# dfdazac/grapes

Measured on AMD Instinct MI355X. Metric: sampled edges aggregated/sec, ogbn-products 3-layer GFlowNet, higher is better.
Workload: dtype f32

## Files before the change

### grapes_amd/_lib.py

```python
from __future__ import annotations

import ctypes as C
import os

_HERE = os.path.dirname(os.path.abspath(__file__))
DIAG_LIB_PATH = os.path.join(_HERE, "libgrapes_hip_diag.so")
DIAG = os.environ.get("GRAPES_DIAG", "0") == "1"
LIB_PATH = os.environ.get("GRAPES_LIB_PATH") or (DIAG_LIB_PATH if DIAG else os.path.join(_HERE, "libgrapes_hip.so"))
ABI_MAJOR, ABI_MINOR = 3, 4


def diag_switch(name: str, default: str) -> str:
    if os.environ.get("GRAPES_DIAG", "0") == "1":
        return os.environ.get(name, default)
    return default


P = C.c_void_p
I32 = C.c_int32
I64 = C.c_int64
U32 = C.c_uint32
U64 = C.c_uint64
F32 = C.c_float
SZ = C.c_size_t
# ... 117 lines not shown
    "grapes_gcn2_mix_fwd": (I32, [P, P, P, F32, F32, F32, I32, P, I32, P, I32, P]),
    "grapes_gcn2_mix_bwd": (I32, [P, P, I32, F32, F32, F32, P, P, P, I32, P, I32, P]),
    "grapes_wgcn_structure_workspace_bytes": (SZ, [I32]),
    "grapes_wgcn_structure": (I32, [P, P, I32, P, I32, P] + [P] * 12),
    "grapes_wgcn_weights": (I32, [P, I32] + [P] * 7 + [I32, P, I32, F32] + [P] * 5),
    "grapes_wgcn_aggregate_workspace_bytes": (SZ, [I32, I32]),
    "grapes_wgcn_aggregate_fwd": (I32, [P] * 8 + [I32, P, I32, I32, I32, P, P, I32, P, P, P]),
    "grapes_wgcn_aggregate_bwd_workspace_bytes": (SZ, [I32, I32, I32, I32]),
    "grapes_wgcn_aggregate_bwd": (I32, [P] * 5 + [I32] + [P] * 14 + [I32, P, I32, I32, P, P, P, P, I32, P, P, P]),
    "grapes_wgcn_loops_workspace_bytes": (SZ, [I32, I32]),
    "grapes_wgcn_loops": (I32, [P, P, I32, P, I32, P, P, P, P, P]),
    "grapes_pna_aggregate_fwd_workspace_bytes": (SZ, [I32, I32]),
    "grapes_pna_aggregate_fwd": (I32, [P, P, P, I32, P, P, P, I32, I32, I32, I32, F32, F32, P, P, I32, P, I32, P, P, I32, P, P, P]),
    "grapes_pna_aggregate_bwd_workspace_bytes": (SZ, [I32, I32, I32]),
    "grapes_pna_aggregate_bwd": (I32, [P, P, I32, P, P, P, P, P, I32, I32, I32, I32, F32, F32, P, P, I32, I32, P, I32, P, P, I32, P, P, P]),
    "grapes_pna_add_input_grad": (I32, [P, P, I32, I32, P, I32, P]),
    "grapes_kernel_clock_enable": (I32, [P, I64]),
    "grapes_kernel_clock_launches": (I32, []),
    "grapes_kernel_clock_entry": (I32, [I32, P, P, P]),
    "grapes_kernel_clock_rate_khz": (I32, []),
    "grapes_gcn_aggregate_fwd_rec": (I32, [P, P, P, P, P, P, P, I32, P, I32, I32, P, P, P, P]),
    "grapes_scatter_rows": (I32, [P, I64, P, P, I64, I32, I32, P, I32, I32, P]),
    "grapes_rider_record_begin": (I32, []),
    "grapes_rider_record_end": (I32, []),
    "grapes_rider_count": (I32, [I32]),
    "grapes_rider_attach": (I32, [I32, I32, P]),
    "grapes_rider_release": (I32, [P]),
    "grapes_rider_detach": (I32, [P, P]),
    "grapes_rider_launch": (I32, [I32, P]),
    "grapes_rider_free": (I32, [I32]),
    "grapes_graph_chain_create": (I32, [P, I32, I32, P, P]),
    "grapes_graph_chain_launch": (I32, [P, P]),
    "grapes_graph_chain_destroy": (I32, [P]),
    "grapes_tensormap_update": (I32, [P, P, I32, P, P]),
    "grapes_tensormap_map": (I32, [P, P, P, I64, P, P]),
    "grapes_frontier_offsets": (I32, [P, P, I32, P, P, P, P]),
    "grapes_frontier_expand": (I32, [P, P, P, I32, P, P, I32, P, P, P, P, P]),
    "grapes_frontier_expand_fused": (I32, [P, P, P, I32, P, I32, P, P, P, P, P, P, P, I32, P, P, P, P, P]),
    "grapes_frontier_expand_fused_ext": (I32, [P, P, P, I32, P, I32, P, P, P, P, P, P, P, I32, P, P, P, P, P, P, P, P, P]),
    "grapes_slice_stage_words": (SZ, [I32]),
    "grapes_bitmap_mark": (I32, [P, P, P, I64, P, I32, P, P]),
    "grapes_bitmap_mark_rows": (I32, [P, P, P, I32, P, P, I32, P, P]),
    "grapes_bitmap_clear": (I32, [P, P, I64, P, P]),
    "grapes_frontier_compact_workspace_bytes": (SZ, [I32, I32]),
    "grapes_frontier_compact": (I32, [P, P, P, I32, I32, P, P, P, P, P, P, U32, P, I32, P, P, SZ, P, SZ, P, SZ, P, P, P, P, P]),
    "grapes_frontier_compact_counted": (I32, [P, P, P, I32, I32, P, P, P, P, P, P, U32, P, I32, P, P, SZ, P, SZ, P, SZ, P, P, P, P, P, P]),
    "grapes_gcn_prepare_counted": (I32, [P, P, P, I32, P, P, I32, P, P, P, P, P, P, P, P, P, P, P, P, P, I64, I32, P, P]),
    "grapes_bitmap_mark_hop": (I32, [P, P, P, P, I32, P, P, P, I32, P, I32, P, P]),
    "grapes_bitmap_mark_lists": (I32, [P, P, P, I32, P, P, I32, P, P, I32, P, P, I32, P, I32, P, P, P]),
    "grapes_union_sorted": (I32, [P, I32, P, P, I32, P, P, I32, P, P, I32, P, I32, I32, P, P, P, P, P, P]),
    "grapes_slice_mark": (I32, [P, P, I32, P, I32, P, P]),
    "grapes_slice_remark": (I32, [P, P, I32, P, P, I32, P, P, P, I32, P, P]),
    "grapes_slice_filter_workspace_bytes": (SZ, [I32]),
    "grapes_slice_filter": (I32, [P, P, P, I32, P, I32, P, P, P, P, P, I32, P, P]),
    "grapes_indicator_mark": (I32, [P, P, I32, P, U32, P, I32, I32, P]),
    "grapes_step_begin": (I32, [P, P, I32, P, I32, P, I32, I32, I32, P, P, I32, I32, P, P]),
    "grapes_gather_rows": (I32, [P, I32, P, I32, P, P, U32, P, I32, P, P]),
    "grapes_gcn_prepare_workspace_bytes": (SZ, [I32, I32]),
    "grapes_gcn_prepare_zero_words": (SZ, [I32]),
    "grapes_gcn_long_items_capacity": (I32, [I32]),
    "grapes_gcn_prepare": (I32, [P, P, I32, P, P, I32, P, I32, P, P, P, P, P, P, P, P, P, P, P, P, P]),
    "grapes_gcn_prepare_prefetching": (I32, [P, P, I32, P, P, I32, P, I32, P, P, P, P, P, P, P, P, P, P, P, P, P, I64, I32, P]),
    "grapes_gcn_prepare_small_batch": (I32, [I32, P, P, P, P, P, I32, P, P, P, P, P, P, P, P, P, P, P, P, P, P, P, P]),
    "grapes_gcn_prepare_from_csr": (I32, [P, I32, P, P, P, I32, P]),
    "grapes_linear_fwd": (I32, [P, P, P, I32, P, I32, I32, P]),
    "grapes_linear_fwd_row_scaled": (I32, [P, P, P, P, I32, P, I32, I32, P]),
    "grapes_eval_predict": (I32, [P, I32, I32, P, P, I32, P, P, P, P]),
    "grapes_linear_bwd_weight_workspace_bytes": (SZ, [I32, I32, I32]),
    "grapes_linear_bwd_weight": (I32, [P, P, P, I32, P, I32, I32, I32, P, P]),
    "grapes_linear_bwd_input": (I32, [P, P, P, I32, P, I32, I32, P]),
    "grapes_linear_bias_act_fwd": (I32, [P, P, P, I32, P, I32, P, I32, I32, P]),
    "grapes_linear_bias_act_head_fwd": (I32, [P, P, P, I32, P, P, P, I32, P, I32, I32, P]),
    "grapes_split_gemm_available": (I32, [I32, I32, I32]),
    "grapes_sampler_head_bwd_multi_workspace_bytes": (SZ, []),
    "grapes_sampler_head_bwd_multi_phase": (I32, [I32, P, P, P, P, P, P, P, P, P, P, P, P, I32, P, P, P, I32, P]),
    "grapes_linear_bias_act_head_fwd_strided": (I32, [P, I32, P, P, I32, P, P, P, I32, P, I32, I32, P]),
    "grapes_linear_bwd_weight_gated_strided": (I32, [P, P, I32, P, I32, P, P, P, P, P, I32, I32, I32, P, P]),
    "grapes_linear_bwd_weight_gated_workspace_bytes": (SZ, [I32, I32, I32]),
    "grapes_linear_bwd_weight_gated": (I32, [P, P, P, P, P, I32, P, I32, I32, I32, P, P, P, P, P]),
    "grapes_linear_bwd_weight_gated_multi": (I32, [I32, P, P, P, P, P, P, P, P, P, I32, I32, I32, P, P]),
    "grapes_linear_bwd_weight_slabs_bytes": (SZ, [I32, I32, I32]),
    "grapes_linear_bwd_weight_slabs": (I32, [P, P, P, I32, P, I32, I32, I32, P, P]),
    "grapes_linear_bwd_weight_slabs_and_input": (I32, [P, P, P, P, P, I32, P, I32, I32, I32, P, P]),
    "grapes_slab_reduce_sets": (I32, [I32, P, P, P, I32, P, I32, P]),
    "grapes_gcn_aggregate_narrow_pair": (I32, [P, P, P, P, P, P, P, P, P, I32, P, P]),
    "grapes_linear_relu_head_fwd_bits": (I32, [P, I32, P, P, P, P, P, I32, P, I32, I32, P]),
    "grapes_linear_relu_head_fwd_bits_pair": (I32, [P, I32, P, P, P, P, P, P, I32, P, P, P, P, P, I32, I32, P, I32, I32, P]),
    "grapes_linear_bwd_weight_bits_multi_cols": (I32, [I32, P, P, P, P, P, P, P, P, P, P, I32, P, P, I32, I32, I32, P, P]),
    "grapes_linear_bwd_weight_bits_pair_cols": (I32, [I32, P, P, P, P, P, P, P, P, P, P, I32, P, P, I32, P, P, P, P, P, P, I32, I32, I32, P, P]),
    "grapes_gcn_aggregate_gather_fwd": (I32, [P, I32, I32, P, P, U32, P, I32, P, P, P, P, P, I32, P, P]),
    "grapes_gcn_aggregate_gather_fwd_peers": (I32, [P, P, I32, I32, I32, P, P, U32, P, I32, P, P, P, P, P, I32, P, P]),
    "grapes_peer_export": (I32, [P, P, P]),
    "grapes_peer_open": (I32, [P, U64, P]),
    "grapes_peer_close": (I32, [P, U64]),
    "grapes_peer_copy": (I32, [P, P, SZ, P]),
    "grapes_gcn_aggregate_workspace_bytes": (SZ, [I32, I32]),
    "grapes_gcn_aggregate_fwd": (I32, [P, P, P, P, P, P, I32, P, I32, I32, P, P, I32, P, P]),
    "grapes_gcn_aggregate_fwd_head": (I32, [P, P, P, P, P, P, I32, P, I32, I32, P, P, P, P]),
    "grapes_gcn_aggregate_fwd_prescaled": (I32, [P, P, P, P, P, P, I32, P, I32, I32, P, P, I32, P, P]),
    "grapes_scale_rows": (I32, [P, P, P, I64, I32, P]),
    "grapes_gcn_aggregate_bwd_rank1_workspace_bytes": (SZ, [I32, I32]),
    "grapes_gcn_aggregate_bwd_rank1": (I32, [P, P, P, P, P, P, P, P, P, I32, I32, P, I32, P, P, I32, P, P]),
    "grapes_gcn_aggregate_bwd_rank1_bits": (I32, [P, P, P, P, P, P, P, P, P, P, I32, I32, P, I32, P, P, I32, P, P]),
    "grapes_gcn_aggregate_bwd_rank1_bits_multi": (I32, [I32, P, P, P, P, P, P, P, P, P, P, P, P, P, I32, P, P, P, P, P]),
    "grapes_gcn_aggregate_bwd_workspace_bytes": (SZ, [I32, I32]),
    "grapes_gcn_aggregate_bwd": (I32, [P, P, P, P, P, P, P, P, I32, I32, P, I32, P, P, I32, P, P, P]),
    "grapes_sampler_workspace_bytes": (SZ, [I32]),
    "grapes_gumbel_topk": (I32, [P, P, P, U64, U64, P, I32, P, I32, I32, P, P, P, P, P, P, P, P, P, I32, P, P, P, P]),
    "grapes_gumbel_topk_hist": (I32, [P, P, P, U64, U64, P, I32, P, I32, I32, P, P, P, P, P, P, P, P, P, I32, P, P, P, P, P]),
    "grapes_gumbel_topk_deferred_ext": (I32, [P, P, P, U64, U64, P, I32, P, I32, I32, P, P, P, P, P, P, P, P, P, I32, P, P, P, P, P, P, P, P, P]),
    "grapes_sampler_hist_words": (I32, []),
    "grapes_gumbel_topk_from_aggregate": (I32, [P, P, P, P, P, P, I32, P, P, P, P, U64, U64, P, I32, P, I32, I32, P, P, P, P, P, P, P, P, P, I32, P, P, P, P]),
    "grapes_bernoulli_logprob_bwd": (I32, [P, P, P, P, P, P, I32, P, P, I32, P, P, P]),
    "grapes_philox_uniform": (I32, [P, I64, U64, U64, P]),
    "grapes_reduce_sum": (I32, [P, I32, P, I32, P, P]),
    "grapes_fill": (I32, [P, I32, P, F32, P, F32, P, I32, P]),
    "grapes_classifier_loss": (I32, [P, I32, I32, P, P, P, P, I32, P, P, P]),
    "grapes_gflownet_loss": (I32, [P, F32, P, I32, I32, P, F32, I32, P, P]),
    "grapes_step_losses_workspace_bytes": (SZ, [I32]),
    "grapes_step_losses": (I32, [P, I32, I32, P, P, P, P, I32, P, P, P, I32, P, F32, P, I32, I32, F32, I32, P, P, P, P, P]),
    "grapes_gcn_aggregate_fwd_losses_available": (I32, [P, P, P, I32, I32]),
    "grapes_gcn_aggregate_fwd_losses": (I32, [P, P, P, P, P, P, I32, P, I32, P, P, P, P, I32, P, P, P, I32, P, F32, P, I32, I32, F32,
                                              I32, P, P, P, P]),
    "grapes_logit_var_reg": (I32, [P, I32, P, I32, F32, P, P, P]),
    "grapes_dropout_fwd": (I32, [P, P, P, I32, P, I32, F32, U64, U64, P, P]),
    "grapes_dropout_bwd": (I32, [P, P, P, I32, P, I32, F32, P]),
    "grapes_adam_desc_bytes": (I32, []),
    "grapes_adam_step": (I32, [P, I32, I64, P, P]),
    "grapes_adam_step_slabs": (I32, [P, I32, I64, P, I32, P, P, I32, P, I32, P]),
    "grapes_exchange_pack_query": (I32, [P, I32, P, I32, P, P]),
    "grapes_exchange_serve_rows": (I32, [P, P, P, I32, I32, I32, I32, P, I64, I32, P, P, P]),
    "grapes_exchange_recv_rows": (I32, [P, I64, P, I32, P, P, I32, I32, P, P, P, P, P, P, P]),
    "grapes_exchange_serve_features": (I32, [P, I32, P, I32, I32, I32, I32, P, I32, P, P]),
    "grapes_exchange_assemble_features": (I32, [P, I32, I32, P, I32, P, P, I32, P, U32, P, I32, P, P]),
    "grapes_exchange_halo_positions": (I32, [P, I32, P, P, I32, I32, P, P, P, P]),
    "grapes_exchange_note_rows": (I32, [P, P, I32, P, P, P, I32, P, P, P, P, I32, P]),
}

_lib = None


DIAG_SIGNATURES = {
    "grapes_debug_gemm_fwd": (I32, [P, P, P, I32, I32, I32, I32, P]),
    "grapes_debug_gather_probe": (I32, [P, I32, P, P, I32, I32, I32, I32, P]),
    "grapes_debug_tsplit_fwd": (I32, [P, I32, I32, P, P, P, I32, I32, I32, P]),
    "grapes_debug_tsplit_dw": (I32, [P, P, I32, I32, P, I32, I32, P, I32, P]),
    "grapes_feature_planes_bytes": (C.c_size_t, [I64, I32]),
    "grapes_feature_split_planes": (I32, [P, I64, I32, P, P]),
    "grapes_feature_planes_register": (I32, [P, I32, P]),
}


class GrapesHipError(RuntimeError):
    pass


_diag_lib = None


def _bind(lib, table, what):
    for name, (res, args) in table.items():
        try:
            fn = getattr(lib, name)
        except AttributeError as e:
            raise GrapesHipError(f"{what} does not export {name}") from e
        fn.restype = res
        fn.argtypes = args


def load_diag():
    global _diag_lib
    if _diag_lib is not None:
        return _diag_lib
    if _lib is not None and LIB_PATH == DIAG_LIB_PATH:
        _diag_lib = _lib
        return _diag_lib
    if not os.path.exists(DIAG_LIB_PATH):
        raise GrapesHipError(f"{DIAG_LIB_PATH} is missing: build it with `make -C grapes_amd/csrc diag`")
    lib = C.CDLL(DIAG_LIB_PATH)
    _bind(lib, SIGNATURES, "libgrapes_hip_diag.so")
    _bind(lib, DIAG_SIGNATURES, "libgrapes_hip_diag.so")
    if lib.grapes_build_flavor() != b"diag":
        raise GrapesHipError("libgrapes_hip_diag.so was not built with -DGRAPES_DIAG")
    _diag_lib = lib
    return lib


def load():
    global _lib
# ... 22 lines not shown
```

### grapes_amd/csrc/common.h

```cpp
#pragma once
#include <hip/hip_runtime.h>
#include <stdint.h>

#include "../../include/grapes_hip.h"

#define GRAPES_WAVE 64
#define DWS_ROWS 128

#define GRAPES_LAUNCH_CHECK()                      \
    do {                                           \
        hipError_t _e = hipGetLastError();         \
        if (_e != hipSuccess) return (int)_e;      \
    } while (0)

static inline int grapes_div_up(int64_t a, int64_t b) { return (int)((a + b - 1) / b); }
static inline bool grapes_aligned16(const void* p) { return (((uintptr_t)p) & 15) == 0; }
static inline size_t grapes_round16(size_t b) { return (b + 15) & ~(size_t)15; }

#include <stdlib.h>
static inline const char* grapes_tune_env(const char* name) {
#ifdef GRAPES_DIAG
    return getenv(name);
#else
    (void)name;
// ... 257 lines not shown
#define GRAPES_STAMP_NW(slot)                                                                                \
    do {                                                                                                     \
        if (grapes_stamp_ptr && threadIdx.x == 0 && blockIdx.x < 64)                                         \
            grapes_stamp_ptr[blockIdx.x * 16 + (slot)] = wall_clock64();                                      \
    } while (0)
#define GRAPES_STAMP_SETTER(name)                                                                            \
    extern "C" int name(unsigned long long* p) {                                                             \
        return (int)hipMemcpyToSymbol(HIP_SYMBOL(grapes_stamp_ptr), &p, sizeof(p));                          \
    }
#else
#define GRAPES_STAMP(slot) do { } while (0)
#define GRAPES_STAMP_NW(slot) do { } while (0)
#define GRAPES_STAMP_SETTER(name)
#endif

#define GRAPES_TS_IMG_ROWS 256

#ifdef __HIPCC__
template <int NT>
__device__ __forceinline__ void draw_stats_final(const double* __restrict__ parts, int blocks, int n, float* __restrict__ stats) {
    __shared__ double ds_red[4][16];
    const int tid = threadIdx.x, lane = tid & 63, wid = tid >> 6;
#pragma unroll
    for (int q = 0; q < 1024 / NT; ++q) {
        double mn = (double)INFINITY, mx = -(double)INFINITY, s1 = 0.0, s2 = 0.0;
        for (int b = tid + NT * q; b < blocks; b += 1024) {
            const long long* p = reinterpret_cast<const long long*>(parts + 5 * (size_t)b);
            mn = fmin(mn, __longlong_as_double(__hip_atomic_load(p + 0, __ATOMIC_RELAXED, __HIP_MEMORY_SCOPE_AGENT)));
            mx = fmax(mx, __longlong_as_double(__hip_atomic_load(p + 1, __ATOMIC_RELAXED, __HIP_MEMORY_SCOPE_AGENT)));
            s1 += __longlong_as_double(__hip_atomic_load(p + 2, __ATOMIC_RELAXED, __HIP_MEMORY_SCOPE_AGENT));
            s2 += __longlong_as_double(__hip_atomic_load(p + 3, __ATOMIC_RELAXED, __HIP_MEMORY_SCOPE_AGENT));
        }
#pragma unroll
        for (int d = 32; d > 0; d >>= 1) {
            mn = fmin(mn, __shfl_xor(mn, d, 64)); mx = fmax(mx, __shfl_xor(mx, d, 64));
            s1 += __shfl_xor(s1, d, 64); s2 += __shfl_xor(s2, d, 64);
        }
        if (lane == 0) { const int vw = wid + (NT / 64) * q; ds_red[0][vw] = mn; ds_red[1][vw] = mx; ds_red[2][vw] = s1; ds_red[3][vw] = s2; }
    }
    __syncthreads();
    if (tid == 0) {
        double mn = (double)INFINITY, mx = -(double)INFINITY, s1 = 0.0, s2 = 0.0;
        for (int w = 0; w < 16; ++w) { mn = fmin(mn, ds_red[0][w]); mx = fmax(mx, ds_red[1][w]); s1 += ds_red[2][w]; s2 += ds_red[3][w]; }
        const double mean = s1 / (double)n;
        double var = n > 1 ? (s2 - s1 * s1 / (double)n) / (double)(n - 1) : 0.0;
        if (var < 0.0) var = 0.0;
        stats[0] = (float)mn; stats[1] = (float)mx; stats[2] = (float)mean; stats[3] = (float)sqrt(var);
    }
}
__device__ __forceinline__ void draw_finish_body(const grapes_draw_finish_args& f) {
    __shared__ double df_red[16];
    const int tid = threadIdx.x, lane = tid & 63, wid = tid >> 6;
    const int n = eff_count(f.d_n, f.n_host);
    const bool keep_all = f.sel[2] != 0u;
    const int nb = keep_all ? f.keys_blocks : (n + f.emit_block - 1) / f.emit_block;
    const double* parts = keep_all ? f.parts_keys : f.parts_emit;
    const int pstride = keep_all ? 5 : 1;
    double v[4];
#pragma unroll
    for (int q = 0; q < 4; ++q) {
        double acc = 0.0;
        for (int bb = tid + 256 * q; bb < nb; bb += 1024) acc += parts[(size_t)bb * pstride];
        v[q] = acc;
    }
#pragma unroll
    for (int q = 0; q < 4; ++q) { const double w = wave_sum_d(v[q]); if (lane == 0) df_red[wid + 4 * q] = w; }
    __syncthreads();
    if (tid == 0 && f.stats) {
        double t = 0.0;
        for (int w = 0; w < 16; ++w) t += df_red[w];
        f.stats[4] = (float)t;
    }
    if (f.hist)
        for (int b = tid; b < f.hist_words; b += 256) f.hist[b] = 0u;
    if (f.stats_blocks > 0 && !keep_all && f.stats) draw_stats_final<256>(f.parts_keys - 4, nb, n, f.stats);
}
#endif

#include <functional>
#include <type_traits>
#include <string.h>
enum GrapesRiderKind { GRAPES_RK_OTHER = 0, GRAPES_RK_EXPAND, GRAPES_RK_COMPACT, GRAPES_RK_FILL, GRAPES_RK_SORT, GRAPES_RK_GATHER,
                       GRAPES_RK_BEGIN ,
                       GRAPES_RK_AGGBWD  };
struct GrapesRiderRecord {
    int kind = GRAPES_RK_OTHER, variant = 0, grid = 0, block = 0;
    size_t arg_bytes = 0;
    alignas(16) unsigned char args[768];
    std::function<void(hipStream_t)> single;
};
bool grapes_rider_recording();
int grapes_rider_grid(int grid);
void grapes_rider_record(GrapesRiderRecord&& r);
#define GRAPES_RIDER_ANY_VARIANT (-0x7fffffff)
const GrapesRiderRecord* grapes_rider_match(int kind, int variant, int block, hipStream_t s);
template <class Args>
static inline GrapesRiderRecord grapes_rider_make(int kind, int variant, int grid, int block, const Args& a,
                                                  std::function<void(hipStream_t)> single) {
    static_assert(sizeof(Args) <= sizeof(GrapesRiderRecord::args), "rider argument block too small");
    static_assert(std::is_trivially_copyable<Args>::value, "rider arguments must be trivially copyable");
    GrapesRiderRecord r;
    r.kind = kind; r.variant = variant; r.grid = grid; r.block = block; r.arg_bytes = sizeof(Args);
    memcpy(r.args, &a, sizeof(Args));
    r.single = std::move(single);
    return r;
}
#define GRAPES_RIDER_OTHER(stream_, launch_expr_)                                                                         \
    do {                                                                                                                  \
        if (grapes_rider_recording()) {                                                                                   \
            GrapesRiderRecord r_;                                                                                         \
            r_.single = [=](hipStream_t s_) { hipStream_t stream_ = s_; (void)stream_; launch_expr_; };                   \
            grapes_rider_record(std::move(r_));                                                                           \
        } else {                                                                                                          \
            launch_expr_;                                                                                                 \
        }                                                                                                                 \
    } while (0)
```

### grapes_amd/csrc/gemm_kernels.hip

```cpp
#include <type_traits>
#include "common.h"
#include <cstdlib>

typedef float f32x16 __attribute__((ext_vector_type(16)));

#define GB_M 128
#define GB_N 128
#define GB_K 16
#define GB_LD 132

struct GatherOp { const int32_t* ids; const uint32_t* code; const uint32_t* d_epoch; uint32_t epoch; int F; uint32_t mask; };

template <bool KMAJOR, bool VEC>
__device__ __forceinline__ void gemm_load_tile(const float* __restrict__ P, long long ld, int r0, int R, int k0,
                                               int kend, int tid, float4 (&v)[2], const float* __restrict__ G = nullptr,
                                               int ones_at = -1, const float* __restrict__ row_scale = nullptr,
                                               const float* __restrict__ col_vec = nullptr, float4* cs2 = nullptr,
                                               const GatherOp* go = nullptr, bool do_cs2 = false) {
    if (VEC) {
#pragma unroll
        for (int i = 0; i < 2; ++i) {
            int k, r;
            bool ok;
            long long off;
// ... 1297 lines not shown
                if (gate && !(gate[o] > 0.f)) v = 0.f;
            }
            As[((k >> 2) * 2 + (k & 1)) * SK_LDA + m * 2 + ((k >> 1) & 1)] = v;
        }
    }
    if (bvec) {
#pragma unroll
        for (int u = 0; u < NB; ++u) {
            const int idx = tid + SK_T * u;
            const int n4 = idx & 15, k = idx >> 4;
            const bool ok = k < kc && n0 + 4 * n4 + 3 < N;
            const float4 v = ok ? vb[u] : make_float4(0.f, 0.f, 0.f, 0.f);
            float* d = &Bs[((k >> 2) * 2 + (k & 1)) * SK_LDB + 8 * n4 + ((k >> 1) & 1)];
            d[0] = v.x; d[2] = v.y; d[4] = v.z; d[6] = v.w;
        }
    } else {
        for (int idx = tid; idx < SK_COLS * DWS_ROWS; idx += SK_T) {
            const int nn = idx & 63, k = idx >> 6;
            const int gn = n0 + nn;
            Bs[((k >> 2) * 2 + (k & 1)) * SK_LDB + nn * 2 + ((k >> 1) & 1)] = (k < kc && gn < N) ? X[(long long)(k0 + k) * ldb + gn] : 0.f;
        }
    }
    __syncthreads();
    {
        const int ct = wid & 1, kqr = wid >> 1;
        constexpr int per = KQ / 4;
        f32x16 acc = {0}, accb = {0};
        const float* Ap = As + h * SK_LDA + li * 2;
        const float* Bp = Bs + h * SK_LDB + (32 * ct + li) * 2;
        const bool colsum = cs_slabs != nullptr && tn == 0 && ct == 0;
        for (int kq = kqr * per; kq < (kqr + 1) * per; ++kq) {
            const float2 a = *reinterpret_cast<const float2*>(Ap + (size_t)kq * 2 * SK_LDA);
            const float2 b = *reinterpret_cast<const float2*>(Bp + (size_t)kq * 2 * SK_LDB);
            acc = __builtin_amdgcn_mfma_f32_32x32x2f32(a.x, b.x, acc, 0, 0, 0);
            acc = __builtin_amdgcn_mfma_f32_32x32x2f32(a.y, b.y, acc, 0, 0, 0);
            if (colsum) {
                accb = __builtin_amdgcn_mfma_f32_32x32x2f32(a.x, 1.0f, accb, 0, 0, 0);
                accb = __builtin_amdgcn_mfma_f32_32x32x2f32(a.y, 1.0f, accb, 0, 0, 0);
            }
        }
        __syncthreads();
#pragma unroll
        for (int r = 0; r < 16; ++r) Ps[((kqr * 2 + ct) * 16 + r) * 64 + lane] = acc[r];
        if (colsum && li == 0) {
#pragma unroll
            for (int r = 0; r < 16; ++r) Pb[kqr][(r & 3) + 8 * (r >> 2) + 4 * h] = accb[r];
        }
    }
    __syncthreads();
    float* C = slabs + (long long)by * M * N;
#pragma unroll
    for (int u = 0; u < 4; ++u) {
        const int o = tid + SK_T * u;
        const int ln = o & 63, r = (o >> 6) & 15, ct = o >> 10;
        const float v0 = Ps[((0 * 2 + ct) * 16 + r) * 64 + ln], v1 = Ps[((1 * 2 + ct) * 16 + r) * 64 + ln];
        const float v2 = Ps[((2 * 2 + ct) * 16 + r) * 64 + ln], v3 = Ps[((3 * 2 + ct) * 16 + r) * 64 + ln];
        const int gn = n0 + 32 * ct + (ln & 31);
        const int gm = m0 + (r & 3) + 8 * (r >> 2) + 4 * (ln >> 5);
        if (gm < M && gn < N) C[(long long)gm * N + gn] = ((v0 + v1) + v2) + v3;
    }
    if (cs_slabs && tn == 0 && tid < SK_ROWS && m0 + tid < M)
        cs_slabs[(long long)by * M + m0 + tid] = ((Pb[0][tid] + Pb[1][tid]) + Pb[2][tid]) + Pb[3][tid];
}
__global__ __launch_bounds__(SK_T) void gemm_dw_small_k(const float* __restrict__ A, const float* __restrict__ gate,
                                                        const float* __restrict__ X, float* __restrict__ slabs,
                                                        float* __restrict__ cs_slabs, int n_host, const int32_t* d_n, int M,
                                                        int N, long long lda, long long ldb) {
    __shared__ __attribute__((aligned(16))) float dws_smem[DWS_SMEM_FLOATS];
    gemm_dw_small_body(A, gate, X, slabs, cs_slabs, n_host, d_n, M, N, lda, ldb, blockIdx.x, blockIdx.y, dws_smem);
}
struct DwSmallArgs { const float* A; const float* gate; const float* X; float* slabs; float* cs_slabs; int M; int N; long long lda; long long ldb; };
struct SkinnyArgs { const float* A; const float* B; float* C; int N; int K; long long lda; long long ldb; long long ldc; };
__global__ __launch_bounds__(SK_T) void gemm_dw_small_dx_pair_k(DwSmallArgs a, SkinnyArgs b, int n_host, const int32_t* d_n,
                                                               int na_x, int na_y, int nb_x) {
    extern __shared__ __attribute__((aligned(16))) float sk_smem[];
    const int id = blockIdx.x, na = na_x * na_y;
    if (id < na) {
        gemm_dw_small_body(a.A, a.gate, a.X, a.slabs, a.cs_slabs, n_host, d_n, a.M, a.N, a.lda, a.ldb, id % na_x, id / na_x, sk_smem);
    } else {
        const int j = id - na;
        gemm_skinny_body<true>(b.A, b.B, b.C, n_host, d_n, b.N, b.K, b.lda, b.ldb, b.ldc, nullptr, 0, j % nb_x, j / nb_x, sk_smem);
    }
}
static inline int dw_nslab(int f_out, int f_in);
static inline bool dw_small_ok(int n, int f_out, int f_in) {
    return n <= 4096 && grapes_div_up(n, DWS_ROWS) <= dw_nslab(f_out, f_in);
}
static int launch_dw_small(const float* a, const float* gate, const float* x, float* slabs, float* cs_slabs, int n,
                           const int32_t* d_n, int f_out, int f_in, long long ldx, hipStream_t s) {
    dim3 grid(grapes_div_up(f_out, SK_ROWS) * grapes_div_up(f_in, SK_COLS), grapes_div_up(n, DWS_ROWS));
    hipLaunchKernelGGL(gemm_dw_small_k, grid, dim3(SK_T), 0, s, a, gate, x, slabs, cs_slabs, n, d_n, f_out, f_in, (long long)f_out, ldx);
    GRAPES_LAUNCH_CHECK();
    return 0;
}

static inline int dw_nslab(int f_out, int f_in) {
    const int tiles = grapes_div_up(f_out, GB_M) * grapes_div_up(f_in, GB_N);
    static int target = 0;
    if (!target) { const char* e = grapes_tune_env("GRAPES_DW_BLOCKS"); target = e ? atoi(e) : 512; if (target < 1) target = 512; }
    int ns = target / tiles;
    return ns < 1 ? 1 : ns;
}

#define SR_MAX_SETS 8
struct SrSets { int nsets; const float* slabs[SR_MAX_SETS]; float* out[SR_MAX_SETS]; long long count[SR_MAX_SETS]; };
__global__ __launch_bounds__(256) void slab_reduce_sets_k(SrSets st, int k_host, const int32_t* d_k, int kchunk, int accumulate) {
    __shared__ float part[4][64];
    const int K = eff_count(d_k, k_host);
    const int ns = (K + kchunk - 1) / kchunk;
    const int g = threadIdx.x >> 6, c = threadIdx.x & 63;
    const int per = (ns + 3) >> 2;
    const int z0 = g * per, z1 = (z0 + per < ns) ? z0 + per : ns;
    long long total = 0;
    for (int q = 0; q < st.nsets; ++q) total += (st.count[q] + 63) & ~63LL;
    for (long long base = (long long)blockIdx.x * 64; base < total; base += (long long)gridDim.x * 64) {
        int q = 0; long long lo = 0;
        for (; q < st.nsets - 1; ++q) { const long long pad = (st.count[q] + 63) & ~63LL; if (base < lo + pad) break; lo += pad; }
        const float* sl = st.slabs[q]; float* o = st.out[q]; const long long cnt = st.count[q];
        const long long i = base - lo + c;
        float acc = 0.f;
        if (i < cnt) {
            int z = z0;
            for (; z + 8 <= z1; z += 8) {
                float v[8];
#pragma unroll
                for (int u = 0; u < 8; ++u) v[u] = sl[(long long)(z + u) * cnt + i];
#pragma unroll
                for (int u = 0; u < 8; ++u) acc += v[u];
            }
            for (; z < z1; ++z) acc += sl[(long long)z * cnt + i];
        }
        part[g][c] = acc;
        __syncthreads();
        if (g == 0 && i < cnt) {
            const float t = (part[0][c] + part[1][c]) + (part[2][c] + part[3][c]);
            o[i] = accumulate ? o[i] + t : t;
        }
        __syncthreads();
    }
}
extern "C" size_t grapes_linear_bwd_weight_slabs_bytes(int32_t n, int32_t f_in, int32_t f_out) {
    const size_t ns = (size_t)grapes_div_up(n > 0 ? n : 1, DWS_ROWS);
    return ns * ((size_t)f_in * f_out + (size_t)f_out) * sizeof(float) + 64;
}
extern "C" int grapes_linear_bwd_weight_slabs(const float* dout, const float* gate, const float* x, int32_t n, const int32_t* d_n,
                                              int32_t f_in, int32_t f_out, int32_t want_bias, void* workspace,
                                              grapes_stream_t stream) {
    if (n <= 0 || f_in <= 0 || f_out <= 1 || !dout || !x || !workspace) return GRAPES_EINVAL;
    if (!dw_small_ok(n, f_out, f_in)) return GRAPES_EINVAL;
    const size_t ns = (size_t)grapes_div_up(n, DWS_ROWS);
    float* w_dw = (float*)workspace;
    float* w_db = w_dw + ns * (size_t)f_in * f_out;
    return launch_dw_small(dout, gate, x, w_dw, want_bias ? w_db : nullptr, n, d_n, f_out, f_in, f_in, (hipStream_t)stream);
}
extern "C" int grapes_linear_bwd_weight_slabs_and_input(const float* dout, const float* gate, const float* x, const float* w,
                                                        float* dx, int32_t n, const int32_t* d_n, int32_t f_in, int32_t f_out,
                                                        int32_t want_bias, void* workspace, grapes_stream_t stream) {
    if (n <= 0 || f_in <= 0 || f_out <= 1 || !dout || !x || !w || !dx || !workspace) return GRAPES_EINVAL;
    if (!dw_small_ok(n, f_out, f_in) || !skinny_ok(n, f_out)) return GRAPES_EINVAL;
    const size_t ns = (size_t)grapes_div_up(n, DWS_ROWS);
    float* w_dw = (float*)workspace;
    float* w_db = w_dw + ns * (size_t)f_in * f_out;
    static bool lds_set = false;
    const size_t lds = ((size_t)SK_KMAX / 4 * 2 * (SK_LDA + SK_LDB) + 4 * 2 * 16 * 64) * sizeof(float);
    if (!lds_set) {
        hipError_t e = hipFuncSetAttribute((const void*)gemm_dw_small_dx_pair_k, hipFuncAttributeMaxDynamicSharedMemorySize, (int)lds);
        if (e != hipSuccess) return (int)e;
        lds_set = true;
    }
    const int KQ = (f_out + 3) / 4;
    size_t lds_use = ((size_t)KQ * 2 * (SK_LDA + SK_LDB) + 4 * 2 * 16 * 64) * sizeof(float);
    if (lds_use < DWS_SMEM_FLOATS * sizeof(float)) lds_use = DWS_SMEM_FLOATS * sizeof(float);
    const int na_x = grapes_div_up(f_out, SK_ROWS) * grapes_div_up(f_in, SK_COLS), na_y = (int)ns;
    const int nb_x = grapes_div_up(n, SK_ROWS), nb_y = grapes_div_up(f_in, SK_COLS);
    DwSmallArgs a{dout, gate, x, w_dw, want_bias ? w_db : nullptr, f_out, f_in, (long long)f_out, (long long)f_in};
    SkinnyArgs b{dout, w, dx, f_in, f_out, (long long)f_out, (long long)f_in, (long long)f_in};
    hipLaunchKernelGGL(gemm_dw_small_dx_pair_k, dim3(na_x * na_y + nb_x * nb_y), dim3(SK_T), lds_use, (hipStream_t)stream, a, b, n, d_n,
                       na_x, na_y, nb_x);
    GRAPES_LAUNCH_CHECK();
    return 0;
}
extern "C" int grapes_slab_reduce_sets(int32_t nsets, const float* const* slabs, float* const* outs, const int64_t* counts,
                                       int32_t n, const int32_t* d_n, int32_t accumulate, grapes_stream_t stream) {
    if (nsets < 1 || nsets > SR_MAX_SETS || !slabs || !outs || !counts || n <= 0) return GRAPES_EINVAL;
    SrSets st; st.nsets = nsets;
    long long total = 0;
    for (int q = 0; q < SR_MAX_SETS; ++q) {
        const int r = q < nsets ? q : 0;
        if (!slabs[r] || !outs[r] || counts[r] <= 0) return GRAPES_EINVAL;
        st.slabs[q] = slabs[r]; st.out[q] = outs[r]; st.count[q] = counts[r];
        if (q < nsets) total += (counts[r] + 63) & ~63LL;
    }
    int grid = (int)(total / 64); if (grid > 8192) grid = 8192; if (grid < 1) grid = 1;
    hipLaunchKernelGGL(slab_reduce_sets_k, dim3(grid), dim3(256), 0, (hipStream_t)stream, st, n, d_n, DWS_ROWS, accumulate);
    GRAPES_LAUNCH_CHECK();
    return 0;
}

extern "C" int grapes_linear_fwd(const float* x, const float* w, float* h, int32_t n, const int32_t* d_n,
                                 int32_t f_in, int32_t f_out, grapes_stream_t stream) {
    if (n < 0 || f_in <= 0 || f_out <= 0) return GRAPES_EINVAL;
    if (n == 0) return 0;
    if (!x || !w || !h) return GRAPES_EINVAL;
    hipStream_t s = (hipStream_t)stream;
    if (f_out == 1) {
        int grid = grapes_div_up(n, 4); if (grid > 8192) grid = 8192;
        hipLaunchKernelGGL(gemv_rows_k, dim3(grid), dim3(256), 0, s, x, w, h, n, d_n, f_in);
        GRAPES_LAUNCH_CHECK();
        return 0;
    }
    if (skinny_ok(n, f_in)) return launch_skinny<false>(x, w, h, n, d_n, f_out, f_in, f_in, f_in, f_out, nullptr, 0, s);
    return launch_gemm<false, false>(x, w, h, n, f_out, f_in, f_in, f_in, f_out, d_n, nullptr, f_in + GB_K, 1, 0, s);
}

__global__ __launch_bounds__(256) void scale_rows_few_k(float* __restrict__ h, const float* __restrict__ sc, int n_host,
                                                        const int32_t* d_n, int f) {
    const int n = eff_count(d_n, n_host);
    const int r = blockIdx.x * 4 + (threadIdx.x >> 6);
    if (r >= n) return;
    const float s = sc[r];
    for (int c = threadIdx.x & 63; c < f; c += 64) h[(long long)r * f + c] *= s;
}

extern "C" int grapes_linear_fwd_row_scaled(const float* x, const float* w, const float* row_scale, float* h, int32_t n,
                                            const int32_t* d_n, int32_t f_in, int32_t f_out, grapes_stream_t stream) {
    if (n < 0 || f_in <= 0 || f_out <= 1) return GRAPES_EINVAL;
    if (n == 0) return 0;
    if (!x || !w || !h || !row_scale) return GRAPES_EINVAL;
    if (skinny_ok(n, f_in)) {
        const int rc = launch_skinny<false>(x, w, h, n, d_n, f_out, f_in, f_in, f_in, f_out, nullptr, 0, (hipStream_t)stream);
        if (rc) return rc;
        hipLaunchKernelGGL(scale_rows_few_k, dim3(grapes_div_up(n, 4)), dim3(256), 0, (hipStream_t)stream, h, row_scale, n, d_n, f_out);
        GRAPES_LAUNCH_CHECK();
        return 0;
    }
    GemmEx ex{};
    ex.out_scale = row_scale;
    return launch_gemm<false, false>(x, w, h, n, f_out, f_in, f_in, f_in, f_out, d_n, nullptr, f_in + GB_K, 1, 0, (hipStream_t)stream, ex);
}

extern "C" size_t grapes_linear_bwd_weight_workspace_bytes(int32_t n_cap, int32_t f_in, int32_t f_out) {
    if (n_cap <= 0) n_cap = 1;
    if (f_out == 1) return grapes_colsum_workspace_bytes(f_in);
    (void)n_cap;
    return (size_t)dw_nslab(f_out, f_in) * f_in * f_out * sizeof(float);
}

extern "C" int grapes_linear_bwd_weight(const float* dh, const float* x, float* dw, int32_t n, const int32_t* d_n,
                                        int32_t f_in, int32_t f_out, int32_t accumulate, void* workspace,
                                        grapes_stream_t stream) {
    if (n < 0 || f_in <= 0 || f_out <= 0 || !dw) return GRAPES_EINVAL;
    hipStream_t s = (hipStream_t)stream;
    if (n == 0) {
        if (!accumulate) { hipError_t e = grapes_zero_async(dw, (size_t)f_in * f_out * sizeof(float), s); if (e) return (int)e; }
        return 0;
    }
    if (!dh || !x || !workspace) return GRAPES_EINVAL;
    if (f_out == 1)
        return grapes_colsum_launch(x, nullptr, dh, nullptr, dw, n, d_n, f_in, accumulate, (float*)workspace, s);
    const int nslab = dw_nslab(f_out, f_in);
    const long long slab = (long long)f_in * f_out;
// ... 1214 lines not shown
```

### grapes_amd/csrc/spmm_kernels.hip

```cpp
#include "common.h"
#include <cstdlib>

template <int VEC>
__device__ __forceinline__ void ld_vec(const float* __restrict__ p, float (&v)[VEC]) {
    if (VEC == 4) {
        const float4 t = *reinterpret_cast<const float4*>(p);
        v[0] = t.x; v[1 % VEC] = t.y; v[2 % VEC] = t.z; v[3 % VEC] = t.w;
    } else {
#pragma unroll
        for (int i = 0; i < VEC; ++i) v[i] = p[i];
    }
}

struct R1 { const float* dh2; const float* w2; };
#define R1_MODE(M) ((M) == 2 || (M) == 4)
template <int VEC, int MODE>
__device__ __forceinline__ void ld_row(const float* __restrict__ h, long long s, int F, int f0, float (&v)[VEC]) {
    if (MODE == 4) {
        const uint32_t wv = reinterpret_cast<const uint32_t*>(h)[8 * s + (f0 >> 5)] >> (f0 & 31);
#pragma unroll
        for (int i = 0; i < VEC; ++i) v[i] = ((wv >> i) & 1u) ? 1.f : 0.f;
    } else {
        ld_vec<VEC>(h + s * F + f0, v);
    }
// ... 1545 lines not shown
        for (int b = 0; b < R; ++b)
            t += __int_as_float(__hip_atomic_load((const int*)(partial + (long long)b * F + c), __ATOMIC_RELAXED, __HIP_MEMORY_SCOPE_AGENT));
        out[c] = accumulate ? out[c] + t : t;
    }
    if (threadIdx.x == 0) ticket[cbx] = 0u;
}

__global__ __launch_bounds__(256) void colsum_ticket_k(const float* __restrict__ src, const float* __restrict__ gate,
                                                       const float* __restrict__ wrow, float* __restrict__ dst,
                                                       float* __restrict__ partial, float* __restrict__ out, int n_host,
                                                       const int32_t* d_n, int F, int accumulate, unsigned* __restrict__ ticket) {
    colsum_ticket_body(src, gate, wrow, dst, partial, out, n_host, d_n, F, accumulate, ticket, blockIdx.x, blockIdx.y, gridDim.y);
}

struct AggBwdSmallArgs {
    const float* dout; const float* gate; const int32_t* rowptr; const int32_t* csr; const float* dinv; float* dh;
    int n_host; const int32_t* d_n; int F; float* dbias; int accumulate_bias; float* partials; unsigned* ticket; int ncb; int R;
};
template <int VEC>
__device__ __forceinline__ void gcn_aggregate_bwd_small_body(const AggBwdSmallArgs& a, int BID, int NBLK) {
    const float* __restrict__ dout = a.dout; const float* __restrict__ gate = a.gate;
    const int32_t* __restrict__ rowptr = a.rowptr; const int32_t* __restrict__ csr = a.csr; const float* __restrict__ dinv = a.dinv;
    float* __restrict__ dh = a.dh;
    const int F = a.F;
    const int ncs = a.dbias ? a.ncb * a.R : 0;
    if (BID < ncs) {
        colsum_ticket_body(dout, gate, nullptr, nullptr, a.partials, a.dbias, a.n_host, a.d_n, F, a.accumulate_bias, a.ticket,
                           BID % a.ncb, BID / a.ncb, a.R);
        return;
    }
    const int n = eff_count(a.d_n, a.n_host);
    const int lane = lane_id();
    const int wave_global = __builtin_amdgcn_readfirstlane(((BID - ncs) * 256 + (int)threadIdx.x) >> 6);
    const int nwaves = ((NBLK - ncs) * 256) >> 6;
    const int f0 = lane * VEC;
    if (f0 >= F) return;
    auto gated = [&](int r, float (&val)[VEC]) {
        ld_vec<VEC>(dout + (long long)r * F + f0, val);
        if (gate) {
            float g[VEC];
            ld_vec<VEC>(gate + (long long)r * F + f0, g);
#pragma unroll
            for (int v = 0; v < VEC; ++v) val[v] = g[v] > 0.f ? val[v] : 0.f;
        }
    };
    for (int row = wave_global; row < n; row += nwaves) {
        const int beg = rowptr[row], end = rowptr[row + 1];
        const float dc = dinv[row];
        float acc[VEC];
#pragma unroll
        for (int v = 0; v < VEC; ++v) acc[v] = 0.f;
        int j = beg;
        for (; j + 4 <= end; j += 4) {
            int s4[4]; float w4[4]; float val[4][VEC];
#pragma unroll
            for (int u = 0; u < 4; ++u) { s4[u] = csr[j + u]; w4[u] = dinv[s4[u]] * dc; }
#pragma unroll
            for (int u = 0; u < 4; ++u) gated(s4[u], val[u]);
#pragma unroll
            for (int u = 0; u < 4; ++u)
#pragma unroll
                for (int v = 0; v < VEC; ++v) acc[v] = fmaf(w4[u], val[u][v], acc[v]);
        }
        for (; j < end; ++j) {
            const int s1 = csr[j];
            const float w1 = dinv[s1] * dc;
            float val[VEC];
            gated(s1, val);
#pragma unroll
            for (int v = 0; v < VEC; ++v) acc[v] = fmaf(w1, val[v], acc[v]);
        }
        float self[VEC];
        gated(row, self);
        float* o = dh + (long long)row * F + f0;
#pragma unroll
        for (int v = 0; v < VEC; ++v) o[v] = fmaf(dc * dc, self[v], acc[v]);
    }
}
template <int VEC>
__global__ __launch_bounds__(256) void gcn_aggregate_bwd_small_k(AggBwdSmallArgs a) {
    gcn_aggregate_bwd_small_body<VEC>(a, (int)blockIdx.x, (int)gridDim.x);
}

size_t grapes_colsum_workspace_bytes(int F) { return (size_t)CS_BLOCKS * (F > 0 ? F : 1) * sizeof(float); }

int grapes_colsum_launch(const float* src, const float* gate, const float* wrow, float* dst, float* out, int n,
                         const int32_t* d_n, int F, int accumulate, float* workspace, hipStream_t s, unsigned* ticket) {
    if (ticket && F > 16 && n <= CS_SMALL_ROWS && grapes_div_up(F, 64) <= 16) {
        int R = grapes_div_up(n, 64); if (R > CS_SMALL_R) R = CS_SMALL_R; if (R < 1) R = 1;
        hipLaunchKernelGGL(colsum_ticket_k, dim3(grapes_div_up(F, 64), R), dim3(256), 0, s, src, gate, wrow, dst, workspace, out, n,
                           d_n, F, accumulate, ticket);
        GRAPES_LAUNCH_CHECK();
        return 0;
    }
    if (F <= 16)
        hipLaunchKernelGGL(colsum_partial_narrow_k, dim3(CS_BLOCKS), dim3(256), 0, s, src, gate, wrow, dst, workspace, n, d_n, F);
    else
        hipLaunchKernelGGL(colsum_partial_k, dim3(CS_BLOCKS), dim3(256), 0, s, src, gate, wrow, dst, workspace, n, d_n, F);
    GRAPES_LAUNCH_CHECK();
    if (out) {
        hipLaunchKernelGGL(colsum_final_k, dim3(grapes_div_up(F, 64)), dim3(256), 0, s, (const float*)workspace, out, F, accumulate);
        GRAPES_LAUNCH_CHECK();
    }
    return 0;
}

extern "C" size_t grapes_gcn_aggregate_workspace_bytes(int32_t item_cap, int32_t f) {
    return (size_t)(item_cap > 0 ? item_cap : 0) * (f > 0 ? f : 1) * sizeof(float) + 16;
}

extern "C" int grapes_gcn_aggregate_fwd(const float* h, const int32_t* rowptr_t, const int32_t* csr_src,
                                        const float* dinv, const float* bias, float* out, int32_t n,
                                        const int32_t* d_n, int32_t f, int32_t relu, const int32_t* long_items,
                                        const int32_t* d_n_items, int32_t item_cap, void* workspace,
                                        grapes_stream_t stream) {
    if (n < 0 || f <= 0) return GRAPES_EINVAL;
    if (n == 0) return 0;
    if (!h || !rowptr_t || !dinv || !out) return GRAPES_EINVAL;
    return launch_aggregate(h, rowptr_t, csr_src, dinv, bias, out, n, d_n, f, relu, long_items, d_n_items, item_cap,
                            (float*)workspace, (hipStream_t)stream);
}

extern "C" int grapes_gcn_aggregate_fwd_losses_available(const float* h, const float* bias, const float* out, int32_t n, int32_t f) {
    const bool vec = (f % 4 == 0) && grapes_aligned16(h) && grapes_aligned16(out) && (!bias || grapes_aligned16(bias));
    return (n > 0 && n <= LOSS_MB_MAXROWS && f > 16 && !vec) ? 1 : 0;
}
extern "C" int grapes_gcn_aggregate_fwd_losses(const float* h, const int32_t* rowptr_t, const int32_t* csr_src, const float* dinv,
                                               const float* bias, float* out, int32_t n, const int32_t* d_n, int32_t f,
                                               const int32_t* node_map, const int32_t* target_ids, const int64_t* labels,
                                               const float* labels_f, int32_t B, float* dlogits, float* loss_out,
                                               const float* z_out, int32_t nz, const int32_t* d_nz, float log_z_init,
                                               const float* hop_stats, int32_t hops, int32_t stats_stride, float loss_coef,
                                               int32_t reinforce, float* out4, void* workspace, uint32_t* d_ticket,
                                               grapes_stream_t stream) {
    if (!h || !rowptr_t || !dinv || !out || !node_map || !target_ids || !dlogits || !loss_out || !out4) return GRAPES_EINVAL;
    if ((labels == nullptr) == (labels_f == nullptr)) return GRAPES_EINVAL;
    if (B <= 0 || B > LOSS_MAX_B || !grapes_gcn_aggregate_fwd_losses_available(h, bias, out, n, f)) return GRAPES_EINVAL;
    if (!hop_stats || hops <= 0 || stats_stride < 5 || nz < 0 || (z_out && nz == 0)) return GRAPES_EINVAL;
    if (!workspace || !d_ticket) return GRAPES_EINVAL;
    if (((uintptr_t)workspace) & 7) return GRAPES_EALIGN;
    const AggregateArgs A{h, rowptr_t, csr_src, dinv, bias, out, n, d_n, f, 0};
    const GfnTail gt{out4, z_out, nz, d_nz, log_z_init, hop_stats, hops, stats_stride, loss_coef, reinforce, nullptr};
    const LossFoldArgs L{node_map, target_ids, labels, labels_f, B, dlogits, loss_out, gt, (float*)workspace, d_ticket};
    const int nA = grapes_div_up(n, 4);
    hipLaunchKernelGGL(gcn_aggregate_losses_k, dim3(nA + 1), dim3(LOSS_MB_THREADS), 0, (hipStream_t)stream, A, L, nA);
    GRAPES_LAUNCH_CHECK();
    return 0;
}

extern "C" int grapes_gcn_aggregate_fwd_head(const float* h, const int32_t* rowptr_t, const int32_t* csr_src, const float* dinv,
                                             const float* bias, float* out, int32_t n, const int32_t* d_n, int32_t f,
                                             int32_t relu, const float* head_w, float* head_out, uint32_t* gate_bits,
                                             grapes_stream_t stream) {
    if (n < 0 || f <= 16 || (f & 3)) return GRAPES_EINVAL;
    if (gate_bits && (f > 256 || !relu)) return GRAPES_EINVAL;
    if (n == 0) return 0;
    if (!h || !rowptr_t || !dinv || !out || !head_w || !head_out) return GRAPES_EINVAL;
    if (!grapes_aligned16(h) || !grapes_aligned16(out) || (bias && !grapes_aligned16(bias)) || !grapes_aligned16(head_w)) return GRAPES_EALIGN;
    int grid = grapes_div_up(n, 4); if (grid > 16384) grid = 16384;
    hipLaunchKernelGGL((gcn_aggregate_k<4, 3>), dim3(grid), dim3(256), 0, (hipStream_t)stream, h, rowptr_t, csr_src, dinv, bias, out,
                       n, d_n, f, relu, 0, f >= 64 ? grapes_clock_reserve("gcn_aggregate_k<4>", grid, 4) : nullptr,
                       R1{nullptr, head_w}, head_out, (uint32_t*)gate_bits);
    GRAPES_LAUNCH_CHECK();
    return 0;
}

// ... 296 lines not shown
        m.dinv[q] = dinv[p]; m.dh[q] = dh[p]; m.n[q] = q < count ? n[p] : 0; m.d_n[q] = d_n[p];
        const bool skip = long_items[p] && d_n_items[p] && item_cap[p] > 0;
        m.items[q] = skip ? long_items[p] : nullptr; m.d_n_items[q] = d_n_items[p]; m.item_cap[q] = skip ? item_cap[p] : 0;
        m.pa[q] = (float*)workspace[p]; m.pb[q] = m.pa[q] + (size_t)CS_BLOCKS * f; m.partials[q] = m.pb[q] + (size_t)CS_BLOCKS * f;
        if (q < count) {
            if (n[p] > nmax) nmax = n[p];
            if (m.item_cap[q] > capmax) capmax = m.item_cap[q];
            if (dw2[p]) {
                any_sum = 1;
                int g = 0;
                for (; g < gr.ngroups; ++g) if (gr.dw2[g] == dw2[p]) break;
                if (g == gr.ngroups) { gr.dw2[g] = dw2[p]; gr.db1[g] = db1[p]; gr.ngroups++; }
                else if (gr.db1[g] != db1[p]) return GRAPES_EINVAL;
                gr.mem[g][gr.nmem[g]] = q; gr.acc[g][gr.nmem[g]] = accumulate[p] ? 1 : 0; gr.nmem[g]++;
            }
        }
    }
    if (any_sum) {
        hipLaunchKernelGGL(colsum_rank1_partial_multi_k, dim3(CS_BLOCKS, count), dim3(256), 0, s, m, f);
        GRAPES_LAUNCH_CHECK();
        hipLaunchKernelGGL(colsum_final2_multi_k, dim3(grapes_div_up(f, 64), 2, gr.ngroups), dim3(256), 0, s, m, gr, f);
        GRAPES_LAUNCH_CHECK();
    }
    static int cap = 0;
    if (!cap) { const char* e = grapes_tune_env("GRAPES_R1BITS_GRID"); cap = e ? atoi(e) : 2048; if (cap < 1) cap = 2048; }
    int gb = grapes_div_up(grapes_div_up(nmax, 4), 4); if (gb > cap) gb = cap;
    hipLaunchKernelGGL(gcn_aggregate_r1bits_multi_k, dim3(gb, count), dim3(256), 0, s, m, f);
    GRAPES_LAUNCH_CHECK();
    if (capmax > 0) {
        const int g2 = capmax < 2048 ? capmax : 2048;
        hipLaunchKernelGGL(gcn_aggregate_chunks_r1bits_multi_k, dim3(g2, count), dim3(256), 0, s, m, f);
        GRAPES_LAUNCH_CHECK();
        hipLaunchKernelGGL(gcn_aggregate_combine_r1bits_multi_k, dim3(g2, count), dim3(256), 0, s, m, f);
        GRAPES_LAUNCH_CHECK();
    }
    return 0;
}

extern "C" size_t grapes_gcn_aggregate_bwd_workspace_bytes(int32_t item_cap, int32_t f) {
    return grapes_colsum_workspace_bytes(f) + grapes_gcn_aggregate_workspace_bytes(item_cap, f);
}

extern "C" int grapes_gcn_aggregate_bwd(const float* dout, const float* relu_out, const int32_t* rowptr_s,
                                        const int32_t* csr_dst, const float* dinv, float* dpre_buf, float* dh,
                                        float* dbias, int32_t accumulate_bias, int32_t n, const int32_t* d_n,
                                        int32_t f, const int32_t* long_items, const int32_t* d_n_items,
                                        int32_t item_cap, void* workspace, uint32_t* d_ticket, grapes_stream_t stream) {
    if (n < 0 || f <= 0) return GRAPES_EINVAL;
    hipStream_t s = (hipStream_t)stream;
    if (n == 0) {
        if (dbias && !accumulate_bias) { hipError_t e = grapes_zero_async(dbias, (size_t)f * sizeof(float), s); if (e) return (int)e; }
        return 0;
    }
    if (!dout || !rowptr_s || !dinv || !dh || !dpre_buf) return GRAPES_EINVAL;
    const bool need_pass = (relu_out != nullptr) || (dbias != nullptr) || (dpre_buf != dout);
    if ((need_pass || long_items) && !workspace) return GRAPES_EINVAL;
    {
        const bool vec = (f % 4 == 0) && grapes_aligned16(dout) && grapes_aligned16(dh) && (!relu_out || grapes_aligned16(relu_out));
        const int VECW = vec ? 4 : 1;
        if (d_ticket && !long_items && n <= CS_SMALL_ROWS && f > 16 && f <= 64 * VECW && grapes_div_up(f, 64) <= 16 && (relu_out || dbias)) {
            const int ncb = grapes_div_up(f, 64);
            int R = grapes_div_up(n, 64); if (R > CS_SMALL_R) R = CS_SMALL_R; if (R < 1) R = 1;
            const int grid = (dbias ? ncb * R : 0) + grapes_div_up(n, 4);
            const AggBwdSmallArgs A{dout, relu_out, rowptr_s, csr_dst, dinv, dh, n, d_n, f, dbias, accumulate_bias, (float*)workspace,
                                    (unsigned*)d_ticket, ncb, R};
            auto single = [=](hipStream_t st) {
                if (vec) hipLaunchKernelGGL((gcn_aggregate_bwd_small_k<4>), dim3(grid), dim3(256), 0, st, A);
                else hipLaunchKernelGGL((gcn_aggregate_bwd_small_k<1>), dim3(grid), dim3(256), 0, st, A);
            };
            if (grapes_rider_recording()) { grapes_rider_record(grapes_rider_make(GRAPES_RK_AGGBWD, VECW, grid, 256, A, single)); return 0; }
            single(s);
            GRAPES_LAUNCH_CHECK();
            return 0;
        }
    }
    if (need_pass) {
        float* dst = (relu_out != nullptr || dpre_buf != dout) ? dpre_buf : nullptr;
        int rc = grapes_colsum_launch(dout, relu_out, nullptr, dst, dbias, n, d_n, f, accumulate_bias, (float*)workspace, s, d_ticket);
        if (rc) return rc;
    }
    float* partials = workspace ? (float*)((char*)workspace + grapes_colsum_workspace_bytes(f)) : nullptr;
    return launch_aggregate(dpre_buf, rowptr_s, csr_dst, dinv, nullptr, dh, n, d_n, f, 0, long_items, d_n_items, item_cap,
                            partials, s);
}


struct BernSegs {
    int count;
    const float* logits[4]; const float* mask[4]; const int32_t* cand_pos[4]; float* dlog[4]; const int32_t* d_n[4]; int n_cap[4];
};
struct BernArgs { const float* d_grad_scale; float* sum_out; int accumulate_sum; float* partials; unsigned* ticket; float* mean_sum_out; };
__device__ __forceinline__ void bernoulli_dense_multi_body(const BernSegs& sg, const BernArgs& ba, int BX, int GX) {
    const float* d_grad_scale = ba.d_grad_scale; float* __restrict__ sum_out = ba.sum_out; const int accumulate_sum = ba.accumulate_sum;
    float* __restrict__ partials = ba.partials; unsigned* __restrict__ ticket = ba.ticket; float* __restrict__ mean_sum_out = ba.mean_sum_out;
    __shared__ float red[4];
    __shared__ int s_last;
    const int q = blockIdx.y;
#define BSEL(f) (q == 0 ? sg.f[0] : (q == 1 ? sg.f[1] : (q == 2 ? sg.f[2] : sg.f[3])))
    const float* logits = BSEL(logits); const float* mask = BSEL(mask); const int32_t* cp = BSEL(cand_pos);
    float* dlog = BSEL(dlog);
    const int n = eff_count(BSEL(d_n), BSEL(n_cap));
#undef BSEL
    const float gs = d_grad_scale ? *d_grad_scale : 1.0f;
    float local = 0.f;
    if (mask == nullptr) {
        const float v = gs * 1.0f / (float)(n > 0 ? n : 1);
        for (int r = BX * 256 + (int)threadIdx.x; r < n; r += GX * 256) dlog[r] = v;
        if (BX == 0 && threadIdx.x == 0 && mean_sum_out) *mean_sum_out = v * (float)n;
    } else {
        for (int r = BX * 256 + (int)threadIdx.x; r < n; r += GX * 256) {
            const int c = cp[r];
            const float l = logits[r];
            float v = 0.f;
            if (c >= 0) v = gs * (mask[c] - 1.0f / (1.0f + expf(-l)));
            dlog[r] = v;
            local += v;
        }
    }
    local = wave_sum(local);
    if (lane_id() == 0) red[threadIdx.x >> 6] = local;
    __syncthreads();
    const unsigned nblk = (unsigned)GX * gridDim.y;
    if (threadIdx.x == 0) {
        publish_f32(&partials[blockIdx.y * GX + BX], (red[0] + red[1]) + (red[2] + red[3]));
        s_last = (atomicAdd(ticket, 1u) == nblk - 1) ? 1 : 0;
    }
    __syncthreads();
    if (!s_last) return;
    float acc = 0.f;
    for (unsigned b = threadIdx.x; b < nblk; b += blockDim.x)
        acc += __int_as_float(__hip_atomic_load((const int*)(partials + b), __ATOMIC_RELAXED, __HIP_MEMORY_SCOPE_AGENT));
    acc = wave_sum(acc);
    __syncthreads();
    if (lane_id() == 0) red[threadIdx.x >> 6] = acc;
    __syncthreads();
    if (threadIdx.x == 0) {
        const float t = (red[0] + red[1]) + (red[2] + red[3]);
        if (sum_out) *sum_out = accumulate_sum ? *sum_out + t : t;
        *ticket = 0u;
    }
}
__global__ __launch_bounds__(256) void bernoulli_dense_multi_k(BernSegs sg, BernArgs ba) {
    bernoulli_dense_multi_body(sg, ba, (int)blockIdx.x, (int)gridDim.x);
}
template <int VEC>
__global__ __launch_bounds__(256) void bernoulli_aggbwd_pair_k(BernSegs sg, BernArgs ba, int gx, AggBwdSmallArgs b) {
    if ((int)blockIdx.x < gx) bernoulli_dense_multi_body(sg, ba, (int)blockIdx.x, gx);
    else {
        const int rx = (int)gridDim.x - gx;
        gcn_aggregate_bwd_small_body<VEC>(b, ((int)blockIdx.x - gx) + (int)blockIdx.y * rx, rx * (int)gridDim.y);
    }
}
template <int VEC>
__global__ __launch_bounds__(256) void narrow_multi_aggbwd_pair_k(NarrowSegs sg, int F, int narrow_lane_rows, int gx, AggBwdSmallArgs b) {
    if ((int)blockIdx.x < gx) {
        const int q = blockIdx.y;
#define NSEL(f) (q == 0 ? sg.f[0] : (q == 1 ? sg.f[1] : (q == 2 ? sg.f[2] : sg.f[3])))
        narrow_body(NSEL(h), NSEL(rowptr), NSEL(csr), NSEL(dinv), NSEL(bias), NSEL(out), NSEL(n_cap), NSEL(d_n), F, 0,
                    narrow_lane_rows, (int)blockIdx.x, gx);
#undef NSEL
    } else {
        const int rx = (int)gridDim.x - gx;
        gcn_aggregate_bwd_small_body<VEC>(b, ((int)blockIdx.x - gx) + (int)blockIdx.y * rx, rx * (int)gridDim.y);
    }
}

extern "C" size_t grapes_sampler_head_bwd_multi_workspace_bytes(void) { return (size_t)4 * 32 * sizeof(float); }

extern "C" int grapes_sampler_head_bwd_multi_phase(int32_t count, const float* const* logits, const float* const* mask,
                                             const int32_t* const* cand_pos, const int32_t* n_cap, const int32_t* const* d_n,
                                             const float* d_grad_scale, const int32_t* const* rowptr_s,
                                             const int32_t* const* csr_dst, const float* const* dinv, float* const* dlogits,
                                             float* const* dh, float* sum_out, int32_t accumulate_sum, float* mean_sum_out,
                                             void* workspace, uint32_t* d_ticket, int32_t phase, grapes_stream_t stream) {
    if (phase < 0 || phase > 2) return GRAPES_EINVAL;
    if (count < 1 || count > 4 || !logits || !mask || !cand_pos || !n_cap || !d_n || !rowptr_s || !csr_dst || !dinv || !dlogits ||
        !dh || !workspace || !d_ticket)
        return GRAPES_EINVAL;
    BernSegs bs{}; NarrowSegs ns{};
    bs.count = ns.count = count;
    int nmax = 0;
    for (int q = 0; q < 4; ++q) {
        const int p = q < count ? q : 0;
        if (q < count && (!rowptr_s[p] || !dinv[p] || !dlogits[p] || !dh[p] || n_cap[p] <= 0)) return GRAPES_EINVAL;
        if (q < count && mask[p] && (!logits[p] || !cand_pos[p])) return GRAPES_EINVAL;
        bs.logits[q] = logits[p]; bs.mask[q] = mask[p]; bs.cand_pos[q] = cand_pos[p]; bs.dlog[q] = dlogits[p]; bs.d_n[q] = d_n[p];
        bs.n_cap[q] = q < count ? n_cap[p] : 0;
        ns.h[q] = dlogits[p]; ns.rowptr[q] = rowptr_s[p]; ns.csr[q] = csr_dst[p]; ns.dinv[q] = dinv[p]; ns.out[q] = dh[p];
        ns.d_n[q] = d_n[p]; ns.n_cap[q] = q < count ? n_cap[p] : 0; ns.bias[q] = nullptr;
        if (q < count && n_cap[p] > nmax) nmax = n_cap[p];
    }
    hipStream_t s = (hipStream_t)stream;
    int g1 = grapes_div_up(nmax, 1024); if (g1 > 32) g1 = 32; if (g1 < 1) g1 = 1;
    auto rider = [&](AggBwdSmallArgs& B, int& vecw, int& rx) -> bool {
        const GrapesRiderRecord* r = grapes_rider_match(GRAPES_RK_AGGBWD, 4, 256, s);
        vecw = 4;
        if (!r) { r = grapes_rider_match(GRAPES_RK_AGGBWD, 1, 256, s); vecw = 1; }
        if (!r) return false;
        memcpy(&B, r->args, sizeof B);
        rx = grapes_div_up(r->grid, count);
        return true;
    };
    AggBwdSmallArgs B; int vecw = 0, rx = 0;
    if (phase != 2) {
        const BernArgs ba{d_grad_scale, sum_out, accumulate_sum, (float*)workspace, (unsigned*)d_ticket, mean_sum_out};
        if (rider(B, vecw, rx)) {
            if (vecw == 4) hipLaunchKernelGGL((bernoulli_aggbwd_pair_k<4>), dim3(g1 + rx, count), dim3(256), 0, s, bs, ba, g1, B);
            else hipLaunchKernelGGL((bernoulli_aggbwd_pair_k<1>), dim3(g1 + rx, count), dim3(256), 0, s, bs, ba, g1, B);
        } else
            hipLaunchKernelGGL(bernoulli_dense_multi_k, dim3(g1, count), dim3(256), 0, s, bs, ba);
        GRAPES_LAUNCH_CHECK();
    }
    if (phase != 1) {
        int g2 = grapes_div_up(nmax, 256); if (g2 > 4096) g2 = 4096;
        if (rider(B, vecw, rx)) {
            if (vecw == 4) hipLaunchKernelGGL((narrow_multi_aggbwd_pair_k<4>), dim3(g2 + rx, count), dim3(256), 0, s, ns, 1, narrow_lane_rows_cfg(), g2, B);
            else hipLaunchKernelGGL((narrow_multi_aggbwd_pair_k<1>), dim3(g2 + rx, count), dim3(256), 0, s, ns, 1, narrow_lane_rows_cfg(), g2, B);
        } else
            hipLaunchKernelGGL(gcn_aggregate_narrow_multi_k, dim3(g2, count), dim3(256), 0, s, ns, 1, narrow_lane_rows_cfg());
        GRAPES_LAUNCH_CHECK();
    }
    return 0;
}
```

### grapes_amd/ops.py

```python
from __future__ import annotations

from typing import List, Optional

import ctypes as _C
import os

import torch

from . import _lib
from ._lib import diag_switch as _sw

_i32 = torch.int32
_i64 = torch.int64
_f32 = torch.float32


def lib():
    return _lib.load()


def _stream() -> int:
    try:
        return torch._C._cuda_getCurrentRawStream(torch._C._cuda_getDevice())
    except AttributeError:
# ... 693 lines not shown
def linear_bwd_weight_gated_strided(x, gate, row_scale, col_vec, dw, dbias=None, dw_head=None, d_n=None, accumulate=False):
    _chk(gate, _f32, "gate"); _chk(row_scale, _f32, "row_scale"); _chk(col_vec, _f32, "col_vec"); _chk(dw, _f32, "dw")
    _chk(dbias, _f32, "dbias", True); _chk(dw_head, _f32, "dw_head", True)
    n, fi = x.shape
    fo = gate.shape[1]
    ldx = _row_strided(x, fi, "linear_bwd_weight_gated_strided")
    ws = _ws(lib().grapes_linear_bwd_weight_gated_workspace_bytes(n, fi, fo), x.device)
    _lib.check(lib().grapes_linear_bwd_weight_gated_strided(_p(gate), x.data_ptr(), ldx, _p(row_scale), n, _p(d_n), _p(col_vec),
                                                            _p(dw), _p(dbias), _p(dw_head), fi, fo, 1 if accumulate else 0,
                                                            _p(ws), _stream()), "linear_bwd_weight_gated_strided")


def linear_bwd_weight_gated(dout, x, gate=None, d_n=None, dw=None, dbias=None, accumulate=False, want_bias=True,
                            row_scale=None, col_vec=None, dw_head=None, defer=None):
    _chk(dw_head, _f32, "dw_head", True)
    _chk(dout, _f32, "dout", row_scale is not None); _chk(x, _f32, "x"); _chk(gate, _f32, "gate", True)
    _chk(row_scale, _f32, "row_scale", True); _chk(col_vec, _f32, "col_vec", True)
    n, fi = x.shape
    fo = dout.shape[1] if dout is not None else gate.shape[1]
    dev = x.device
    if dw is None:
        dw = torch.empty((fo, fi), dtype=_f32, device=dev)
        accumulate = False
    if want_bias and dbias is None:
        dbias = torch.empty(fo, dtype=_f32, device=dev)
    if (defer is not None and row_scale is None and dout is not None and fo > 1 and
            defer.try_add(dout, gate, x, d_n, dw, dbias if want_bias else None, accumulate)):
        return dw, dbias
    ws = _ws(lib().grapes_linear_bwd_weight_gated_workspace_bytes(n, fi, fo), dev)
    _lib.check(lib().grapes_linear_bwd_weight_gated(_p(dout), _p(gate), _p(x), _p(dw), _p(dbias) if want_bias else None, n,
                                                    _p(d_n), fi, fo, 1 if accumulate else 0, _p(row_scale), _p(col_vec),
                                                    _p(dw_head), _p(ws), _stream()),
               "linear_bwd_weight_gated")
    return dw, dbias


def linear_bwd_weight_gated_multi(gates, xs, row_scales, d_ns, col_vec, dw, dbias=None, dw_head=None, accumulate=False):
    import ctypes as C
    nseg = len(gates)
    if not (1 <= nseg <= 4 and len(xs) == nseg and len(row_scales) == nseg and len(d_ns) == nseg):
        raise ValueError("1..4 hops with matching operand lists")
    for t in list(gates) + list(xs) + list(row_scales) + [col_vec, dw]:
        _chk(t, _f32, "operand")
    fo, fi = gates[0].shape[1], xs[0].shape[1]
    arr = lambda ts: (C.c_void_p * nseg)(*[t.data_ptr() for t in ts])
    caps = (C.c_int32 * nseg)(*[x.shape[0] for x in xs])
    ws = _ws(lib().grapes_linear_bwd_weight_gated_workspace_bytes(1, fi, fo), dw.device)
    _lib.check(lib().grapes_linear_bwd_weight_gated_multi(nseg, arr(gates), arr(xs), arr(row_scales), arr(d_ns), caps,
                                                          _p(col_vec), _p(dw), _p(dbias), _p(dw_head), fi, fo,
                                                          1 if accumulate else 0, _p(ws), _stream()),
               "linear_bwd_weight_gated_multi")
    return dw


class DeferredSlabs:

    def __init__(self):
        self.sets, self.n, self.d_n, self.acc = [], None, None, None

    def try_add(self, dout, gate, x, d_n, dw, dbias, accumulate, w=None, dx=None):
        n, fi = x.shape
        fo = dout.shape[1]
        if len(self.sets) + (2 if dbias is not None else 1) > 8:
            self.flush()
        if self.sets and (self.n != n or (self.d_n is None) != (d_n is None) or
                          (d_n is not None and self.d_n.data_ptr() != d_n.data_ptr()) or self.acc != bool(accumulate)):
            self.flush()
        ws = _ws(lib().grapes_linear_bwd_weight_slabs_bytes(n, fi, fo), x.device)
        if dx is not None:
            rc = lib().grapes_linear_bwd_weight_slabs_and_input(_p(dout), _p(gate), _p(x), _p(w), _p(dx), n, _p(d_n), fi, fo,
                                                                1 if dbias is not None else 0, _p(ws), _stream())
        else:
            rc = lib().grapes_linear_bwd_weight_slabs(_p(dout), _p(gate), _p(x), n, _p(d_n), fi, fo, 1 if dbias is not None else 0,
                                                      _p(ws), _stream())
        if rc != 0:
            return False
        ns = (n + 127) // 128
        self.n, self.d_n, self.acc = n, d_n, bool(accumulate)
        self.sets.append((ws, ws.data_ptr(), dw, fo * fi))
        if dbias is not None:
            self.sets.append((ws, ws.data_ptr() + ns * fo * fi * 4, dbias, fo))
        return True

    def flush(self):
        if not self.sets:
            return
        import ctypes as C
        k = len(self.sets)
        slabs = (C.c_void_p * k)(*[s[1] for s in self.sets])
        outs = (C.c_void_p * k)(*[s[2].data_ptr() for s in self.sets])
        counts = (C.c_int64 * k)(*[s[3] for s in self.sets])
        _lib.check(lib().grapes_slab_reduce_sets(k, slabs, outs, counts, self.n, _p(self.d_n), 1 if self.acc else 0, _stream()),
                   "slab_reduce_sets")
        self.sets = []


class GateBits:
    __slots__ = ("words", "n", "f_out")

    def __init__(self, words, n, f_out):
        self.words, self.n, self.f_out = words, n, f_out


def linear_relu_head_fwd_bits(x, w, bias, head_w, d_n=None):
    _chk(w, _f32, "w"); _chk(bias, _f32, "bias", True); _chk(head_w, _f32, "head_w")
    n, fi = x.shape
    fo = w.shape[0]
    ldx = _row_strided(x, fi, "linear_relu_head_fwd_bits")
    words = torch.empty((n, (fo + 31) // 32), dtype=torch.int32, device=x.device)
    head = torch.empty((n, 1), dtype=_f32, device=x.device)
    _lib.check(lib().grapes_linear_relu_head_fwd_bits(x.data_ptr(), ldx, _p(w), _p(bias), _p(head_w), _p(words), _p(head), n,
                                                      _p(d_n), fi, fo, _stream()), "linear_relu_head_fwd_bits")
    return GateBits(words, n, fo), head


def _dw_cols(dw, fo, fi, what):
    if dw.dim() != 2 or dw.shape[0] != fo or not dw.is_contiguous() or not (fi - 3 <= dw.shape[1] <= fi):
        raise ValueError(f"{what}: dw must be a dense [f_out, f_in] matrix (or [f_out, K], f_in = K rounded up to a multiple of 4)")
    return int(dw.shape[1])


def linear_bwd_weight_bits_multi(bits, xs, row_scales, d_ns, col_vec, w1, b1, dw, dbias=None, dw_head=None, accumulate=False):
    import ctypes as C
    nseg = len(bits)
    if not (1 <= nseg <= 4 and len(xs) == nseg and len(row_scales) == nseg and len(d_ns) == nseg):
        raise ValueError("1..4 row sets with matching operand lists")
    for t in list(row_scales) + [col_vec, dw, w1, b1]:
        _chk(t, _f32, "operand")
    fo, fi = bits[0].f_out, xs[0].shape[1]
    if tuple(w1.shape) != (fo, fi) or not w1.is_contiguous() or b1.numel() != fo:
        raise ValueError("linear_bwd_weight_bits_multi: w1 must be a dense [f_out, f_in] matrix and b1 [f_out]")
    dw_cols = _dw_cols(dw, fo, fi, "linear_bwd_weight_bits_multi")
    strides = (C.c_int32 * nseg)(*[_row_strided(x, fi, "linear_bwd_weight_bits_multi") for x in xs])
    arr = lambda ts: (C.c_void_p * nseg)(*[t.data_ptr() for t in ts])
    caps = (C.c_int32 * nseg)(*[x.shape[0] for x in xs])
    ws = _ws(lib().grapes_linear_bwd_weight_gated_workspace_bytes(1, fi, fo), dw.device)
    _lib.check(lib().grapes_linear_bwd_weight_bits_multi_cols(nseg, arr([b.words for b in bits]), arr(xs), strides, arr(row_scales),
                                                              arr(d_ns), caps, _p(col_vec), _p(w1), _p(b1), _p(dw), dw_cols,
                                                              _p(dbias), _p(dw_head), fi, fo, 1 if accumulate else 0, _p(ws),
                                                              _stream()),
               "linear_bwd_weight_bits_multi")
    return dw


def linear_bwd_weight_bits_pair(bits, xs, row_scales, d_ns, col_vec, w1, b1, dw, dbias, dw_head,
                                bits_b, x_b, row_scale_b, d_n_b, col_vec_b, w1_b, b1_b, dw_b, dbias_b, dw_head_b, accumulate=False):
    import ctypes as C
    nseg = len(bits)
    if not (1 <= nseg <= 3 and len(xs) == nseg and len(row_scales) == nseg and len(d_ns) == nseg):
        raise ValueError("1..3 row sets of layer a with matching operand lists")
    for t in list(row_scales) + [row_scale_b, col_vec, col_vec_b, dw, dw_b, w1, b1, w1_b, b1_b]:
        _chk(t, _f32, "operand")
    fo, fi, fib = bits[0].f_out, xs[0].shape[1], x_b.shape[1]
    if (bits_b.f_out != fo or tuple(w1.shape) != (fo, fi) or tuple(w1_b.shape) != (fo, fib) or not w1.is_contiguous() or
            not w1_b.is_contiguous()):
        raise ValueError("linear_bwd_weight_bits_pair: dense [f_out, f_in] weights of one f_out")
    allx = list(xs) + [x_b]
    strides = (C.c_int32 * (nseg + 1))(*[_row_strided(x, fi if i < nseg else fib, "linear_bwd_weight_bits_pair") for i, x in enumerate(allx)])
    arr = lambda ts: (C.c_void_p * (nseg + 1))(*[t.data_ptr() for t in ts])
    caps = (C.c_int32 * (nseg + 1))(*[x.shape[0] for x in allx])
    ws = _ws(lib().grapes_linear_bwd_weight_gated_workspace_bytes(1, fi, fo), dw.device)
    dw_cols = _dw_cols(dw, fo, fi, "linear_bwd_weight_bits_pair")
    _lib.check(lib().grapes_linear_bwd_weight_bits_pair_cols(
        nseg, arr([b.words for b in bits] + [bits_b.words]), arr(allx), strides, arr(list(row_scales) + [row_scale_b]),
        arr(list(d_ns) + [d_n_b]), caps, _p(col_vec), _p(w1), _p(b1), _p(dw), dw_cols, _p(dbias), _p(dw_head), fi,
        _p(col_vec_b), _p(w1_b), _p(b1_b), _p(dw_b), _p(dbias_b), _p(dw_head_b), fib, fo, 1 if accumulate else 0, _p(ws),
# ... 293 lines not shown
            _p(prep.n_items_s) if use_items else None, prep.item_cap if use_items else 0, _p(ws), _stream()),
            "gcn_aggregate_bwd_rank1_bits")
        return dh
    _lib.check(lib().grapes_gcn_aggregate_bwd_rank1(_p(act), _p(dh2), _p(w2), _p(prep.rowptr_s), _p(prep.csr_dst), _p(prep.dinv),
                                                    _p(dh), _p(dw_head), _p(dbias), 1 if accumulate else 0, n, _p(prep.d_n), f,
                                                    _p(prep.items_s) if use_items else None,
                                                    _p(prep.n_items_s) if use_items else None,
                                                    prep.item_cap if use_items else 0, _p(ws), _stream()),
               "gcn_aggregate_bwd_rank1")
    return dh


def gcn_aggregate_bwd_rank1_multi(problems):
    import ctypes as C
    k = len(problems)
    if not (1 <= k <= 3):
        raise ValueError("gcn_aggregate_bwd_rank1_multi: 1..3 problems")
    f = problems[0]["act"].shape[1]
    dev = problems[0]["act"].device
    dhs, wss, ns, caps, items, nitems, accs = [], [], [], [], [], [], []
    for pr in problems:
        act, dh2, w2, prep, bits = pr["act"], pr["dh2"], pr["w2"], pr["prep"], pr["gate_bits"]
        _chk(act, _f32, "act"); _chk(dh2, _f32, "dh2"); _chk(w2, _f32, "w2")
        _chk(pr.get("dw_head"), _f32, "dw_head", True); _chk(pr.get("dbias"), _f32, "dbias", True)
        n = act.shape[0]
        if act.shape[1] != f or dh2.numel() != n or w2.numel() != f or f > 256:
            raise ValueError("gcn_aggregate_bwd_rank1_multi: one width f <= 256; dh2 [n], w2 [f]")
        if bits is None or bits.dtype != _i32 or tuple(bits.shape) != (n, 8) or not bits.is_contiguous():
            raise ValueError("gcn_aggregate_bwd_rank1_multi: gate_bits int32 [n, 8]")
        use_items = prep.n > _SMALL_GRAPH
        dhs.append(torch.empty_like(act))
        wss.append(_ws(lib().grapes_gcn_aggregate_bwd_rank1_workspace_bytes(prep.item_cap, f), dev))
        ns.append(n); caps.append(prep.item_cap if use_items else 0)
        items.append(prep.items_s if use_items else None); nitems.append(prep.n_items_s if use_items else None)
        accs.append(1 if pr.get("accumulate") else 0)
    arr = lambda ts: (C.c_void_p * k)(*[None if t is None else t.data_ptr() for t in ts])
    ints = lambda vs: (C.c_int32 * k)(*vs)
    _lib.check(lib().grapes_gcn_aggregate_bwd_rank1_bits_multi(
        k, arr([p["act"] for p in problems]), arr([p["gate_bits"] for p in problems]), arr([p["dh2"] for p in problems]),
        arr([p["w2"] for p in problems]), arr([p["prep"].rowptr_s for p in problems]), arr([p["prep"].csr_dst for p in problems]),
        arr([p["prep"].dinv for p in problems]), arr(dhs), arr([p.get("dw_head") for p in problems]),
        arr([p.get("dbias") for p in problems]), ints(accs), ints(ns), arr([p["prep"].d_n for p in problems]), f, arr(items),
        arr(nitems), ints(caps), arr(wss), _stream()), "gcn_aggregate_bwd_rank1_bits_multi")
    return dhs


def scale_rows(h, dinv, out=None):
    _chk(h, _f32, "h"); _chk(dinv, _f32, "dinv")
    n, f = h.shape
    if out is None:
        out = torch.empty_like(h)
    _lib.check(lib().grapes_scale_rows(_p(h), _p(dinv), _p(out), n, f, _stream()), "scale_rows")
    return out


def gcn_aggregate_fwd_prescaled(hs, prep: PreparedGraph, bias=None, relu=False, out=None):
    _chk(hs, _f32, "hs"); _chk(bias, _f32, "bias", True)
    n, f = hs.shape
    if out is None:
        out = torch.empty_like(hs)
    use_items = prep.items_fwd and prep.n > _SMALL_GRAPH
    ws = _ws(lib().grapes_gcn_aggregate_workspace_bytes(prep.item_cap, f), hs.device) if use_items else None
    _lib.check(lib().grapes_gcn_aggregate_fwd_prescaled(_p(hs), _p(prep.rowptr_t), _p(prep.csr_src), _p(prep.dinv), _p(bias),
                                                        _p(out), n, _p(prep.d_n), f, 1 if relu else 0,
                                                        _p(prep.items_t) if use_items else None,
                                                        _p(prep.n_items_t) if use_items else None,
                                                        prep.item_cap if use_items else 0, _p(ws), _stream()),
               "gcn_aggregate_fwd_prescaled")
    return out


def gcn_aggregate_narrow_pair(h_a, h_b, prep: PreparedGraph, bias_a=None, bias_b=None):
    _chk(h_a, _f32, "h_a"); _chk(h_b, _f32, "h_b"); _chk(bias_a, _f32, "bias_a", True); _chk(bias_b, _f32, "bias_b", True)
    if h_a.numel() != h_b.numel():
        raise ValueError("gcn_aggregate_narrow_pair: two vectors of one length")
    out_a, out_b = torch.empty_like(h_a), torch.empty_like(h_b)
    _lib.check(lib().grapes_gcn_aggregate_narrow_pair(_p(h_a), _p(h_b), _p(prep.rowptr_t), _p(prep.csr_src), _p(prep.dinv),
                                                      _p(bias_a), _p(bias_b), _p(out_a), _p(out_b), h_a.numel(), _p(prep.d_n),
                                                      _stream()), "gcn_aggregate_narrow_pair")
    return out_a, out_b


_BWD_HOSTS: List = []


def carry_backward_aggregations(hosts):
    _BWD_HOSTS[:] = list(hosts)


def flush_backward_hosts():
    while _BWD_HOSTS:
        _BWD_HOSTS.pop(0)()


def gcn_aggregate_bwd(dout, prep: PreparedGraph, relu_out=None, want_bias=True, dbias=None, accumulate_bias=False):
    _chk(dout, _f32, "dout"); _chk(relu_out, _f32, "relu_out", True)
    n, f = dout.shape
    dev = dout.device
    dpre = torch.empty_like(dout) if relu_out is not None else dout
    dh = torch.empty_like(dout)
    if want_bias and dbias is None:
        dbias = torch.empty(f, dtype=_f32, device=dev)
        accumulate_bias = False
    ws = _ws(lib().grapes_gcn_aggregate_bwd_workspace_bytes(prep.item_cap, f), dev)
    use_items = prep.n > _SMALL_GRAPH
    L = lib()
    host = _BWD_HOSTS.pop(0) if (_BWD_HOSTS and not use_items) else None
    if host is not None:
        _lib.check(L.grapes_rider_record_begin(), "rider_record_begin")
    prog = -1
    try:
        rc = L.grapes_gcn_aggregate_bwd(_p(dout), _p(relu_out), _p(prep.rowptr_s), _p(prep.csr_dst), _p(prep.dinv),
                                        _p(dpre), _p(dh), _p(dbias) if want_bias else None,
                                        1 if accumulate_bias else 0, n, _p(prep.d_n), f,
                                        _p(prep.items_s) if use_items else None,
                                        _p(prep.n_items_s) if use_items else None,
                                        prep.item_cap if use_items else 0, _p(ws), _p(_ticket(dev)[16:32]), _stream())
    finally:
        if host is not None:
            prog = int(L.grapes_rider_record_end())
    _lib.check(rc, "gcn_aggregate_bwd")
    if host is not None:
        _lib.check(L.grapes_rider_attach(prog, 0, _stream()), "rider_attach")
        try:
            host()
        finally:
            alone = L.grapes_rider_detach(_stream(), None)
            L.grapes_rider_free(prog)
        if alone < 0:
            raise _lib.GrapesHipError(f"rider_detach failed ({alone})")
    return dh, dbias


def gather_width_ok(f: int, wide_scalar: bool = False) -> bool:
    return 1 <= f <= 1024 and (wide_scalar or f <= 256 or f % 4 == 0)


def _gather_width(f: int, who: str, wide_scalar: bool = False):
    if not gather_width_ok(f, wide_scalar):
        built = "any width up to 1024" if wide_scalar else "any width up to 256, multiples of 4 up to 1024"
        raise ValueError(f"{who}: width {f} is not built ({built})")


def _long_items(prep, by_target: bool, forward: bool, long_rows: Optional[bool] = None):
    small = prep.n <= _SMALL_GRAPH if long_rows is None else not long_rows
    if small or (forward and not prep.items_fwd):
        return None, None, 0
    items, n_items = (prep.items_t, prep.n_items_t) if by_target else (prep.items_s, prep.n_items_s)
    return _p(items), _p(n_items), prep.item_cap


def gat_scores(h, a_src, a_dst, d_n=None):
    _chk(h, _f32, "h"); _chk(a_src, _f32, "a_src"); _chk(a_dst, _f32, "a_dst")
    n, f = h.shape
    _gather_width(f, "GAT aggregation")
    if a_src.numel() != f or a_dst.numel() != f:
        raise ValueError("a_src / a_dst must hold one value per column of h")
    s_src = torch.empty(max(n, 1), dtype=_f32, device=h.device)
    s_dst = torch.empty(max(n, 1), dtype=_f32, device=h.device)
    _lib.check(lib().grapes_gat_scores(_p(h), _p(a_src), _p(a_dst), _p(s_src), _p(s_dst), n, _p(d_n), f, _stream()), "gat_scores")
    return s_src, s_dst


def gat_aggregate_fwd(h, s_src, s_dst, prep: PreparedGraph, bias=None, relu=False, out=None):
    _chk(h, _f32, "h"); _chk(s_src, _f32, "s_src"); _chk(s_dst, _f32, "s_dst"); _chk(bias, _f32, "bias", True)
    n, f = h.shape
    _gather_width(f, "GAT aggregation")
    if n != prep.n or s_src.numel() < n or s_dst.numel() < n:
        raise ValueError("h, s_src and s_dst need one row per node of the prepared graph")
    if out is None:
        out = torch.empty_like(h)
    row_ms = torch.empty((max(n, 1), 2), dtype=_f32, device=h.device)
    items, n_items, cap = _long_items(prep, by_target=True, forward=True)
    ws = _ws(lib().grapes_gat_aggregate_workspace_bytes(cap, f), h.device) if cap else None
    _lib.check(lib().grapes_gat_aggregate_fwd(_p(h), _p(s_src), _p(s_dst), _p(prep.rowptr_t), _p(prep.csr_src), _p(bias), _p(out),
                                              _p(row_ms), n, _p(prep.d_n), f, 1 if relu else 0, items, n_items, cap, _p(ws),
                                              _p(prep.status), _stream()), "gat_aggregate_fwd")
    return out, row_ms


def gat_aggregate_bwd(dout, out, h, s_src, s_dst, row_ms, a_src, a_dst, prep: PreparedGraph, bias=None, relu=False):
    for t, name in ((dout, "dout"), (out, "out"), (h, "h"), (s_src, "s_src"), (s_dst, "s_dst"), (row_ms, "row_ms"),
                    (a_src, "a_src"), (a_dst, "a_dst")):
        _chk(t, _f32, name)
    _chk(bias, _f32, "bias", True)
    n, f = dout.shape
    _gather_width(f, "GAT aggregation")
    if n != prep.n or out.shape != dout.shape or h.shape != dout.shape:
        raise ValueError("dout, out and h must be [n, f] over the prepared graph's nodes")
    dev = dout.device
    dh = torch.empty_like(dout)
    da_src = torch.empty(f, dtype=_f32, device=dev); da_dst = torch.empty(f, dtype=_f32, device=dev)
    dbias = torch.empty(f, dtype=_f32, device=dev)
    items_t, n_items_t, cap = _long_items(prep, by_target=True, forward=False)
    items_s, n_items_s, _ = _long_items(prep, by_target=False, forward=False)
    ws = _ws(lib().grapes_gat_aggregate_bwd_workspace_bytes(n, cap, f), dev)
    _lib.check(lib().grapes_gat_aggregate_bwd(_p(dout), _p(out), _p(bias), 1 if relu else 0, _p(h), _p(s_src), _p(s_dst), _p(row_ms),
                                              _p(a_src), _p(a_dst), _p(prep.rowptr_t), _p(prep.csr_src), _p(prep.rowptr_s),
                                              _p(prep.csr_dst), _p(dh), _p(da_src), _p(da_dst), _p(dbias), n, _p(prep.d_n), f,
                                              items_t, n_items_t, items_s, n_items_s, cap, _p(ws), _p(prep.status), _stream()),
               "gat_aggregate_bwd")
    return dh, da_src, da_dst, dbias


def _gatv2_shape(heads: int, c: int):
    if not 1 <= heads <= 16:
        raise ValueError(f"GATv2 aggregation: heads = {heads} is not built (1 <= heads <= 16)")
    f = heads * c
    if c < 1 or f > 1024 or (f > 256 and c % 4):
        raise ValueError(f"GATv2 aggregation: heads x out_channels = {heads} x {c} is not built (heads * out_channels up to 256, "
                         "or up to 1024 with out_channels % 4 == 0)")


def _gatv2_slope(negative_slope: float) -> float:
# ... 2177 lines not shown
```

### grapes_amd/step_graph.py

```python
from __future__ import annotations

import contextlib
import copy
from typing import Dict, List, Optional

import os

import torch

from ._lib import diag_switch as _sw
import torch.nn as nn

from . import ops
from .capture import SegmentedGraph
from .graph import DeviceGraph


class _FirstLayer:

    def __init__(self, conv, F, num_ind, legacy=False):
        self.conv, self.F, self.num_ind = conv, F, num_ind
        self.K = F + num_ind
        self.Kp = self.K if legacy else (self.K + 3) // 4 * 4
        self.agg_first = legacy or self.K < conv.out_channels or conv.out_channels % 4 != 0
# ... 690 lines not shown
            preps = ops.PreparedGraph.small_batch(s.slices, self.nall_cap, d_n=d_na, status=st, node_map=g.node_map,
                                                  head_ids=hid, counters=self._ctr[hops:], stages=s.stages if s.staged else None)
        else:
            preps = [ops.PreparedGraph(ksrc, kdst, self.nall_cap, d_n=d_na, d_e=kcnt, status=st, src_grouped=True,
                                       node_map=g.node_map, head_ids=hid, counters=self._ctr[hops + i])
                     for i, (ksrc, kdst, kcnt) in enumerate(s.slices)]
        layers = list(self.gcn_c.gcn_layers)
        s.alln, s.d_na, s.preps, s.layers = alln, d_na, preps, layers
        s.used = [preps[-i] for i in range(1, len(layers))] + [preps[0]]
        s.first_relu = len(layers) > 1
        s.first_fused = (not self.partitioned) or (len(layers) > 1 and self.F < layers[0].out_channels)

    def _classifier_forward(self, s):
        layers, used, alln, d_na = s.layers, s.used, s.alln, s.d_na
        pdrop = self.dropout
        keeps: List[Optional[torch.Tensor]] = []

        def drop(t):
            if not pdrop:
                keeps.append(None)
                return t
            y, keep = ops.dropout_fwd(t, pdrop, philox_seed=self.seed, d_philox_offset=self.philox_off, d_n=d_na)
            keeps.append(keep)
            return y
        x_rows = self.g.rows_from_kept(s.kept_halo, alln, d_na) if (s.halo_reuse and s.kept_halo is not None) else None
        if s.first_fused:
            xc, a1 = self._first_fwd(s, layers[0], alln, used[0], 0, self.epoch_t, relu=s.first_relu, x_rows=x_rows)
            acts = [xc, drop(a1)]
        elif x_rows is not None:
            acts = [x_rows]
        else:
            acts = [self.g.assemble(self.g.fetch_halo(alln, d_n=d_na))]
        fold = (not pdrop and not self.reg_param and not self.evaluate and _sw("GRAPES_LOSS_FOLD", "1") != "0")
        for li in range(len(acts) - 1, len(layers)):
            if fold and li == len(layers) - 1:
                logits, s.losses = self._conv_fwd_losses(s, layers[li], acts[-1], used[li])
                acts.append(drop(logits))
                break
            acts.append(drop(self._conv_fwd(layers[li], acts[-1], used[li], li < len(layers) - 1)))
        for p in used:
            i = self.hops + next(i for i, q in enumerate(s.preps) if q is p)
            s.agg_w[i] += 1
            s.agg_x[i] += 1
        s.acts, s.keeps, s.logits = acts, keeps, acts[-1]

    def _conv_fwd_losses(self, s, conv, x, prep):
        rnd = self.random_sampling
        h = ops.linear_fwd(x, conv.lin.weight, d_n=prep.d_n)
        r = ops.gcn_aggregate_fwd_losses(h, prep, conv.bias, self.g.node_map, self.targets, self.y, s.hop_stats, self.loss_coef,
                                         z_out=None if rnd else s.zstate["zout"].view(-1),
                                         d_nz=None if rnd else s.zstate["d_nb"],
                                         log_z_init=self.log_z_init, reinforce=self.reinforce)
        if r is None:
            return ops.gcn_aggregate_fwd(h, prep, conv.bias, False), None
        return r[0], r

    def _eval_outputs(self, s):
        g = self.g
        pred, rows = ops.eval_predict(s.logits, g.node_map, self.targets, status=g.status)
        self.out = dict(pred=pred if self.y.dim() == 1 else (rows > 0), target_logits=rows, n_all=s.d_na,
                        all_nodes=s.alln, logits=s.logits, kept=[k for k, _ in s.kept_list], kept_counts=[c for _, c in s.kept_list],
                        sizes=s.dnn_list, agg_counts=self._ctr[:, 2], agg_weights=tuple(s.agg_w), agg_executed=tuple(s.agg_x),
                        hop_logits=[hs["logit"] for hs in s.hop_state], nb_local=s.nbl_list, neighbor_nodes=s.neigh_list)

    def _losses(self, s):
        rnd, logits, d_na = self.random_sampling, s.logits, s.d_na
        if s.losses is not None:
            _, s.loss_c, s.dl, out4 = s.losses
            s.loss_gfn, s.gscale, s.log_z, s.tot = out4[0], out4[1:2], out4[2], out4[3]
            return
        reg_term = ops.logit_var_reg(logits, self.reg_param, d_n=d_na) if self.reg_param else None
        s.loss_c, s.dl, out4 = ops.step_losses(logits, self.g.node_map, self.targets, self.y, s.hop_stats, self.loss_coef,
                                               z_out=None if rnd else s.zstate["zout"].view(-1),
                                               d_nz=None if rnd else s.zstate["d_nb"],
                                               log_z_init=self.log_z_init, reinforce=self.reinforce, loss_extra=reg_term)
        if self.reg_param:
            ops.logit_var_reg(logits, self.reg_param, d_n=d_na, dlogits=s.dl)
        s.loss_gfn, s.gscale, s.log_z, s.tot = out4[0], out4[1:2], out4[2], out4[3]

    def _classifier_backward(self, s):
        layers, acts, used, keeps, alln, d_na = s.layers, s.acts, s.used, s.keeps, s.alln, s.d_na
        d = s.dl
        deferred = ops.DeferredSlabs() if _sw("GRAPES_DEFER_SLABS", "1") != "0" else None
        for i in range(len(layers) - 1, -1, -1):
            if keeps[i] is not None:
                d = ops.dropout_bwd(d, keeps[i], self.dropout, d_n=d_na)
            if i == 0 and s.first_fused:
                self._first_bwd(layers[0], acts[0], acts[1], d, used[0], False, relu=s.first_relu, defer=deferred)
                if self.embed:
                    fl0 = self._fl[id(layers[0])]
                    if not fl0.agg_first:
                        raise NotImplementedError("embedding gradient through a transform-first classifier layer")
                    t, _ = ops.gcn_aggregate_bwd(d, used[0], relu_out=acts[1] if s.first_relu else None, want_bias=False)
                    dxr = ops.linear_bwd_input(t, fl0.weight, d_n=used[0].d_n)
                    ops.scatter_rows(self.X.grad, alln, dxr, d_n=d_na, F=self.F)
            else:
                d = self._conv_bwd(layers[i], acts[i], acts[i + 1], d, used[i], i < len(layers) - 1, i > 0, False,
                                   defer=deferred)
        if deferred is not None:
            if (self.grad_sync is None and self._fused_adam is not False and self.opt_c is not None and
                    not any(fl.publishes for fl in self._fl.values()) and not self.reinforce and
                    _sw("GRAPES_ADAM_SLABS", "1") != "0"):
                self._pending_slabs = deferred
            else:
                deferred.flush()

    def _backward(self, s):
        rnd = self.random_sampling
        fork = (not rnd) and _sw("GRAPES_BWD_FORK", "0") != "0"
        if fork:
            main_s = torch.cuda.current_stream()
            if self._side is None:
                self._side = torch.cuda.Stream()
            self._side.wait_stream(main_s)
            with torch.cuda.stream(self._side):
                self._classifier_backward(s)
        carry_bwd = (not fork) and (not self.embed) and _sw("GRAPES_BWD_CARRY", "1") != "0"
        cb_done = (not rnd) and self._nets_backward(s, carry_bwd)
        if fork:
            main_s.wait_stream(self._side)
        elif not cb_done:
            self._classifier_backward(s)

    def _nets_backward(self, s, carry_bwd) -> bool:
        hops, num_ind, ep = self.hops, self.num_ind, self.epoch_t
        gf1, gf2, st_gf, z1, z2, st_z = self._nets()
        hop_state, zstate, gscale = s.hop_state, s.zstate, s.gscale
        z_done = False
        cb_done = False
        fi_, fo_ = st_gf.Kp, gf1.out_channels
        multi = hops <= 4 and st_gf.agg_first and fi_ % 4 == 0 and fi_ % 128 != 0 and fo_ % 4 == 0
        heads = multi or (hops <= 4 and all(hs.get("cand_pos") is not None for hs in hop_state) and
                          _sw("GRAPES_HEAD_BWD_MULTI", "1") != "0")
        dh2s, z_dh2 = None, None
        if heads:
            z_rides = (not self.reinforce) and hops <= 3
            zs = [zstate] if z_rides else []
            hb = ops.SamplerHeadBwdMulti([hs["logit"].view(-1) for hs in hop_state] + [z["zout"].view(-1) for z in zs],
                                         [hs["mask"] for hs in hop_state] + [None for _ in zs],
                                         [hs["cand_pos"] for hs in hop_state] + [None for _ in zs],
                                         [hs["prep"] for hs in hop_state] + [z["prep"] for z in zs],
                                         d_grad_scale=gscale, sum_out=gf2.bias.grad, accumulate_sum=False,
                                         mean_sum_out=z2.bias.grad if z_rides else None)
            if carry_bwd:
                if self._rider_end_hook is not None:
                    self._rider_end_hook()
                ops.carry_backward_aggregations([lambda: hb.launch(1), lambda: hb.launch(2)])
                try:
                    self._classifier_backward(s)
                finally:
                    ops.flush_backward_hosts()
                cb_done = True
            else:
                hb.launch(0)
            dh2_all = hb.dh
            dh2s = [dh2_all[h][:hs["logit"].numel()] for h, hs in enumerate(hop_state)]
            z_dh2 = dh2_all[hops][:zstate["zout"].numel()].view(-1, 1) if z_rides else None
        if multi:
            if all(isinstance(hs["act1"], ops.GateBits) for hs in hop_state):
                if (z_dh2 is not None and isinstance(zstate["act"], ops.GateBits) and hops <= 3 and
                        zstate["x"].shape[1] <= st_gf.Kp and _sw("GRAPES_DW_PAIR", "1") != "0"):
                    ops.linear_bwd_weight_bits_pair(
                        [hs["act1"] for hs in hop_state], [hs["x"] for hs in hop_state], dh2s, [hs["prep"].d_n for hs in hop_state],
                        gf2.lin.weight.view(-1), st_gf.weight, gf1.bias, st_gf.grad_direct, gf1.bias.grad, gf2.lin.weight.grad.view(-1),
                        zstate["act"], zstate["x"], z_dh2.view(-1), zstate["prep"].d_n, z2.lin.weight.view(-1), st_z.weight, z1.bias,
                        st_z.grad, z1.bias.grad, z2.lin.weight.grad.view(-1), accumulate=False)
                    z_done = True
                else:
                    ops.linear_bwd_weight_bits_multi([hs["act1"] for hs in hop_state], [hs["x"] for hs in hop_state], dh2s,
                                                     [hs["prep"].d_n for hs in hop_state], gf2.lin.weight.view(-1), st_gf.weight,
                                                     gf1.bias, st_gf.grad_direct, dbias=gf1.bias.grad,
                                                     dw_head=gf2.lin.weight.grad.view(-1), accumulate=False)
            else:
                ops.linear_bwd_weight_gated_multi([hs["act1"] for hs in hop_state], [hs["x"] for hs in hop_state], dh2s,
                                                  [hs["prep"].d_n for hs in hop_state], gf2.lin.weight.view(-1),
                                                  st_gf.grad, dbias=gf1.bias.grad,
                                                  dw_head=gf2.lin.weight.grad.view(-1), accumulate=False)
        dh_r1s, z_r1 = [None] * len(hop_state), None
        if (dh2s is not None and not multi and _sw("GRAPES_R1_MULTI", "1") != "0" and
                all(self._r1_ok(gf1, hs["act1"]) for hs in hop_state)):
            z_in = (z_dh2 is not None and not (self.reinforce or z_done) and self._r1_ok(z1, zstate["act"]) and
# ... 376 lines not shown
```

### include/grapes_hip.h

```cpp
#ifndef GRAPES_HIP_H
#define GRAPES_HIP_H

#include <stddef.h>
#include <stdint.h>

#ifdef __cplusplus
extern "C" {
#endif

#define GRAPES_ABI_VERSION 304

#define GRAPES_EINVAL (-1)
#define GRAPES_EALIGN (-2)

#define GRAPES_STATUS_EDGE_OVERFLOW 1
#define GRAPES_STATUS_NODE_OVERFLOW 2
#define GRAPES_STATUS_BAD_INDEX 4
#define GRAPES_STATUS_SYNC_TIMEOUT 8
#define GRAPES_SYNC_WORDS 256

typedef void* grapes_stream_t;

int grapes_abi_version(void);
const char* grapes_target_arch(void);
// ... 102 lines not shown
                        int32_t* node_map, int32_t* counts, int32_t* unmark_mult, int32_t* status, grapes_stream_t stream);

int grapes_slice_mark(int32_t* mult, const int32_t* cols, int32_t c, const int32_t* d_c,
                      int32_t unmark, uint64_t* clear_bits, grapes_stream_t stream);
int grapes_slice_remark(int32_t* mult, const int32_t* unmark_ids, int32_t n_unmark, const int32_t* d_n_unmark,
                        const int32_t* mark_ids, int32_t n_mark, const int32_t* d_n_mark, uint64_t* clear_bits,
                        const int32_t* clear_ids, int32_t n_clear, const int32_t* d_n_clear, grapes_stream_t stream);
size_t grapes_slice_filter_workspace_bytes(int32_t e_cap);
int grapes_slice_filter(const int32_t* mult, const int32_t* src, const int32_t* dst, int32_t e,
                        const int32_t* d_e, int32_t out_cap, int32_t* out_src, int32_t* out_dst,
                        int32_t* d_out_count, void* workspace, uint64_t* sync, int32_t counted, int32_t* status,
                        grapes_stream_t stream);

int grapes_indicator_mark(uint32_t* ind_code, const int32_t* ids, int32_t n, const int32_t* d_n,
                          uint32_t epoch, uint32_t* d_epoch, int32_t bit, int32_t advance_epoch,
                          grapes_stream_t stream);
int grapes_step_begin(uint32_t* ind_code, uint32_t* d_epoch, int32_t bit, const int32_t* ids, int32_t n_ids,
                      int32_t* d_cursor, int32_t stride, int32_t offset, int32_t batch, int32_t* targets,
                      const int32_t* counters, int32_t counter_stride, int32_t n_counters, int64_t* totals,
                      grapes_stream_t stream);
int grapes_gather_rows(const float* X, int32_t F, const int32_t* ids, int32_t n,
                       const int32_t* d_n, const uint32_t* ind_code, uint32_t epoch,
                       const uint32_t* d_epoch,
                       int32_t num_ind, float* out, grapes_stream_t stream);

#define GRAPES_PREP_SRC_GROUPED 1
#define GRAPES_PREP_PREZEROED 2
#define GRAPES_LONG_ROW 64
size_t grapes_gcn_prepare_workspace_bytes(int32_t n_cap, int32_t e_cap);
int32_t grapes_gcn_long_items_capacity(int32_t e_cap);
size_t grapes_gcn_prepare_zero_words(int32_t n);
int grapes_gcn_prepare(const int32_t* edge_src, const int32_t* edge_dst, int32_t e,
                       const int32_t* d_e, const int32_t* node_map, int32_t n, const int32_t* d_n, int32_t flags,
                       int32_t* rowptr_t, int32_t* csr_src, int32_t* rowptr_s, int32_t* csr_dst,
                       float* dinv, int32_t* long_items, int32_t* n_long, const int32_t* head_ids,
                       int32_t* row_head, void* workspace, uint64_t* sync, int32_t* status, grapes_stream_t stream);
int grapes_gcn_prepare_prefetching(const int32_t* edge_src, const int32_t* edge_dst, int32_t e, const int32_t* d_e,
                                   const int32_t* node_map, int32_t n, const int32_t* d_n, int32_t flags,
                                   int32_t* rowptr_t, int32_t* csr_src, int32_t* rowptr_s, int32_t* csr_dst,
                                   float* dinv, int32_t* long_items, int32_t* n_long, const int32_t* head_ids,
                                   int32_t* row_head, void* workspace, uint64_t* sync, int32_t* status, const float* prefetch_X,
                                   int64_t prefetch_pitch, int32_t prefetch_row_floats, grapes_stream_t stream);

int grapes_gcn_prepare_small_batch(int32_t count, const int32_t* const* edge_src, const int32_t* const* edge_dst,
                                   const int32_t* e, const int32_t* const* d_e, const int32_t* node_map,
                                   int32_t n, const int32_t* d_n, int32_t* const* rowptr_t,
                                   int32_t* const* csr_src, int32_t* const* rowptr_s, int32_t* const* csr_dst,
                                   float* const* dinv, int32_t* const* long_items, int32_t* const* n_long,
                                   const int32_t* head_ids, int32_t* const* row_head, void* const* workspaces,
                                   const int32_t* const* slice_stage, const int32_t* const* d_fe, const int32_t* fe_cap,
                                   int32_t* status, grapes_stream_t stream);

int grapes_gcn_prepare_from_csr(const int32_t* rowptr, int32_t n, float* dinv, int32_t* items,
                                int32_t* n_items, int32_t item_cap, grapes_stream_t stream);

int grapes_linear_fwd(const float* x, const float* w, float* h, int32_t n, const int32_t* d_n,
                      int32_t f_in, int32_t f_out, grapes_stream_t stream);
int grapes_linear_fwd_row_scaled(const float* x, const float* w, const float* row_scale, float* h, int32_t n,
                                 const int32_t* d_n, int32_t f_in, int32_t f_out, grapes_stream_t stream);
size_t grapes_linear_bwd_weight_workspace_bytes(int32_t n_cap, int32_t f_in, int32_t f_out);
int grapes_linear_bwd_weight(const float* dh, const float* x, float* dw, int32_t n,
                             const int32_t* d_n, int32_t f_in, int32_t f_out, int32_t accumulate,
                             void* workspace, grapes_stream_t stream);
int grapes_linear_bias_act_fwd(const float* x, const float* w, const float* bias, int32_t relu,
                               float* out, int32_t n, const int32_t* d_n, int32_t f_in,
                               int32_t f_out, grapes_stream_t stream);
int grapes_linear_bias_act_head_fwd(const float* x, const float* w, const float* bias, int32_t relu, float* out,
                                    const float* head_w, float* head_out, int32_t n, const int32_t* d_n,
                                    int32_t f_in, int32_t f_out, grapes_stream_t stream);
int32_t grapes_split_gemm_available(int32_t n, int32_t f_in, int32_t f_out);
int grapes_linear_bias_act_head_fwd_strided(const float* x, int32_t x_stride, const float* w, const float* bias,
                                            int32_t relu, float* out, const float* head_w, float* head_out, int32_t n,
                                            const int32_t* d_n, int32_t f_in, int32_t f_out, grapes_stream_t stream);
int grapes_linear_bwd_weight_gated_strided(const float* gate, const float* x, int32_t x_stride, const float* row_scale,
                                           int32_t n, const int32_t* d_n, const float* col_vec, float* dw, float* dbias,
                                           float* dw_head, int32_t f_in, int32_t f_out, int32_t accumulate,
                                           void* workspace, grapes_stream_t stream);
size_t grapes_linear_bwd_weight_slabs_bytes(int32_t n, int32_t f_in, int32_t f_out);
int grapes_linear_bwd_weight_slabs(const float* dout, const float* gate, const float* x, int32_t n, const int32_t* d_n,
                                   int32_t f_in, int32_t f_out, int32_t want_bias, void* workspace, grapes_stream_t stream);
int grapes_linear_bwd_weight_slabs_and_input(const float* dout, const float* gate, const float* x, const float* w, float* dx,
                                             int32_t n, const int32_t* d_n, int32_t f_in, int32_t f_out, int32_t want_bias,
                                             void* workspace, grapes_stream_t stream);
int grapes_slab_reduce_sets(int32_t nsets, const float* const* slabs, float* const* outs, const int64_t* counts, int32_t n,
                            const int32_t* d_n, int32_t accumulate, grapes_stream_t stream);
int grapes_linear_relu_head_fwd_bits(const float* x, int32_t x_stride, const float* w, const float* bias,
                                     const float* head_w, uint32_t* gate_bits, float* head_out, int32_t n,
                                     const int32_t* d_n, int32_t f_in, int32_t f_out, grapes_stream_t stream);
int grapes_linear_relu_head_fwd_bits_pair(const float* x, int32_t x_stride, const float* w, const float* bias,
                                          const float* head_w, uint32_t* gate_bits, float* head_out,
                                          const float* x_b, int32_t x_stride_b, const float* w_b, const float* bias_b,
                                          const float* head_w_b, uint32_t* gate_bits_b, float* head_out_b, int32_t f_in_b,
                                          int32_t n, const int32_t* d_n, int32_t f_in, int32_t f_out, grapes_stream_t stream);
int grapes_linear_bwd_weight_bits_multi_cols(int32_t nseg, const uint32_t* const* gate_bits, const float* const* x,
                                             const int32_t* x_stride, const float* const* row_scale,
                                             const int32_t* const* d_n, const int32_t* n_cap, const float* col_vec,
                                             const float* w1, const float* b1, float* dw, int32_t dw_cols, float* dbias,
                                             float* dw_head, int32_t f_in, int32_t f_out, int32_t accumulate, void* workspace,
                                             grapes_stream_t stream);
int grapes_linear_bwd_weight_bits_pair_cols(int32_t nseg, const uint32_t* const* gate_bits, const float* const* x,
                                            const int32_t* x_stride, const float* const* row_scale,
                                            const int32_t* const* d_n, const int32_t* n_cap, const float* col_vec,
                                            const float* w1, const float* b1, float* dw, int32_t dw_cols, float* dbias,
                                            float* dw_head, int32_t f_in, const float* col_vec_b, const float* w1_b,
                                            const float* b1_b, float* dw_b, float* dbias_b, float* dw_head_b, int32_t f_in_b,
                                            int32_t f_out, int32_t accumulate, void* workspace, grapes_stream_t stream);
size_t grapes_linear_bwd_weight_gated_workspace_bytes(int32_t n_cap, int32_t f_in, int32_t f_out);
int grapes_linear_bwd_weight_gated(const float* dout, const float* gate, const float* x, float* dw,
                                   float* dbias, int32_t n, const int32_t* d_n, int32_t f_in,
                                   int32_t f_out, int32_t accumulate, const float* row_scale,
                                   const float* col_vec, float* dw_head, void* workspace, grapes_stream_t stream);
int grapes_linear_bwd_weight_gated_multi(int32_t nseg, const float* const* gate, const float* const* x,
                                         const float* const* row_scale, const int32_t* const* d_n,
                                         const int32_t* n_cap, const float* col_vec, float* dw, float* dbias,
                                         float* dw_head, int32_t f_in, int32_t f_out, int32_t accumulate,
                                         void* workspace, grapes_stream_t stream);
#ifdef GRAPES_DIAG
int grapes_debug_gemm_fwd(const float* x, const float* w, float* out, int32_t n, int32_t f_in,
                          int32_t f_out, int32_t dbg, grapes_stream_t stream);
int grapes_debug_gather_probe(const float* X, int32_t x_stride, const int32_t* row_head, float* out, int32_t n,
                              int32_t f_out, int32_t variant, int32_t grid_cap, grapes_stream_t stream);
int grapes_debug_tsplit_fwd(const float* X, int32_t F, int32_t x_stride, const int32_t* ids, const void* w_image, float* h,
                            int32_t n, int32_t f_out, int32_t dbg, grapes_stream_t stream);
int grapes_debug_tsplit_dw(const float* dh, const float* X, int32_t F, int32_t x_stride, const int32_t* ids, int32_t n,
                           int32_t f_out, void* workspace, int32_t dbg, grapes_stream_t stream);
#endif
int grapes_linear_bwd_input(const float* dh, const float* w, float* dx, int32_t n,
                            const int32_t* d_n, int32_t f_in, int32_t f_out,
                            grapes_stream_t stream);
size_t grapes_gcn_aggregate_workspace_bytes(int32_t item_cap, int32_t f);
int grapes_gcn_aggregate_narrow_pair(const float* h_a, const float* h_b, const int32_t* rowptr_t, const int32_t* csr_src,
                                     const float* dinv, const float* bias_a, const float* bias_b, float* out_a, float* out_b,
                                     int32_t n, const int32_t* d_n, grapes_stream_t stream);
int grapes_gcn_aggregate_fwd(const float* h, const int32_t* rowptr_t, const int32_t* csr_src,
                             const float* dinv, const float* bias, float* out, int32_t n,
                             const int32_t* d_n, int32_t f, int32_t relu,
                             const int32_t* long_items, const int32_t* d_n_items, int32_t item_cap,
                             void* workspace, grapes_stream_t stream);
int grapes_gcn_aggregate_fwd_head(const float* h, const int32_t* rowptr_t, const int32_t* csr_src, const float* dinv,
                                  const float* bias, float* out, int32_t n, const int32_t* d_n, int32_t f, int32_t relu,
                                  const float* head_w, float* head_out, uint32_t* gate_bits, grapes_stream_t stream);
int grapes_gcn_aggregate_fwd_losses_available(const float* h, const float* bias, const float* out, int32_t n, int32_t f);
int grapes_gcn_aggregate_fwd_losses(const float* h, const int32_t* rowptr_t, const int32_t* csr_src, const float* dinv,
                                    const float* bias, float* out, int32_t n, const int32_t* d_n, int32_t f,
                                    const int32_t* node_map, const int32_t* target_ids, const int64_t* labels,
                                    const float* labels_f, int32_t B, float* dlogits, float* loss_out, const float* z_out,
                                    int32_t nz, const int32_t* d_nz, float log_z_init, const float* hop_stats, int32_t hops,
                                    int32_t stats_stride, float loss_coef, int32_t reinforce, float* out4, void* workspace,
                                    uint32_t* d_ticket, grapes_stream_t stream);
int grapes_gcn_aggregate_fwd_rec(const float* h, const int32_t* row_head, const int32_t* rowptr_t, const int32_t* csr_src,
                                 const float* dinv, const float* bias, float* out, int32_t n, const int32_t* d_n, int32_t f,
                                 int32_t relu, const float* head_w, float* head_out, uint32_t* gate_bits, grapes_stream_t stream);
int grapes_gcn_aggregate_fwd_prescaled(const float* hs, const int32_t* rowptr_t, const int32_t* csr_src,
                                       const float* dinv, const float* bias, float* out, int32_t n,
                                       const int32_t* d_n, int32_t f, int32_t relu, const int32_t* long_items,
                                       const int32_t* d_n_items, int32_t item_cap, void* workspace,
                                       grapes_stream_t stream);
size_t grapes_gcn_aggregate_bwd_rank1_workspace_bytes(int32_t item_cap, int32_t f);
int grapes_gcn_aggregate_bwd_rank1(const float* act, const float* dh2, const float* w2, const int32_t* rowptr_s,
                                   const int32_t* csr_dst, const float* dinv, float* dh, float* dw2, float* db1,
                                   int32_t accumulate, int32_t n, const int32_t* d_n, int32_t f,
                                   const int32_t* long_items, const int32_t* d_n_items, int32_t item_cap,
                                   void* workspace, grapes_stream_t stream);
int grapes_gcn_aggregate_bwd_rank1_bits(const float* act, const uint32_t* gate_bits, const float* dh2, const float* w2,
                                        const int32_t* rowptr_s, const int32_t* csr_dst, const float* dinv, float* dh,
                                        float* dw2, float* db1, int32_t accumulate, int32_t n, const int32_t* d_n,
                                        int32_t f, const int32_t* long_items, const int32_t* d_n_items, int32_t item_cap,
                                        void* workspace, grapes_stream_t stream);
int grapes_gcn_aggregate_bwd_rank1_bits_multi(int32_t count, const float* const* act, const uint32_t* const* gate_bits,
                                              const float* const* dh2, const float* const* w2, const int32_t* const* rowptr_s,
                                              const int32_t* const* csr_dst, const float* const* dinv, float* const* dh,
                                              float* const* dw2, float* const* db1, const int32_t* accumulate, const int32_t* n,
                                              const int32_t* const* d_n, int32_t f, const int32_t* const* long_items,
                                              const int32_t* const* d_n_items, const int32_t* item_cap, void* const* workspace,
                                              grapes_stream_t stream);
int grapes_scale_rows(const float* h, const float* dinv, float* hs, int64_t n, int32_t f, grapes_stream_t stream);
int grapes_gcn_aggregate_gather_fwd(const float* X, int32_t F, int32_t x_stride, const int32_t* ids,
                                    const uint32_t* ind_code, uint32_t epoch, const uint32_t* d_epoch,
                                    int32_t num_ind, const int32_t* rowptr_t, const int32_t* csr_src,
                                    const float* dinv, const int32_t* row_head, float* out, int32_t n,
                                    const int32_t* d_n, grapes_stream_t stream);
size_t grapes_gcn_aggregate_bwd_workspace_bytes(int32_t item_cap, int32_t f);
#define GRAPES_COLSUM_TICKETS 16
int grapes_gcn_aggregate_bwd(const float* dout, const float* relu_out, const int32_t* rowptr_s,
                             const int32_t* csr_dst, const float* dinv, float* dpre_buf,
                             float* dh, float* dbias, int32_t accumulate_bias, int32_t n,
                             const int32_t* d_n, int32_t f, const int32_t* long_items,
                             const int32_t* d_n_items, int32_t item_cap, void* workspace,
                             uint32_t* d_ticket, grapes_stream_t stream);

int grapes_gat_scores(const float* h, const float* a_src, const float* a_dst, float* s_src, float* s_dst, int32_t n,
                      const int32_t* d_n, int32_t f, grapes_stream_t stream);
size_t grapes_gat_aggregate_workspace_bytes(int32_t item_cap, int32_t f);
int grapes_gat_aggregate_fwd(const float* h, const float* s_src, const float* s_dst, const int32_t* rowptr_t,
                             const int32_t* csr_src, const float* bias, float* out, float* row_ms, int32_t n,
                             const int32_t* d_n, int32_t f, int32_t relu, const int32_t* long_items,
                             const int32_t* d_n_items, int32_t item_cap, void* workspace, int32_t* status,
                             grapes_stream_t stream);
size_t grapes_gat_aggregate_bwd_workspace_bytes(int32_t n, int32_t item_cap, int32_t f);
int grapes_gat_aggregate_bwd(const float* dout, const float* out, const float* bias, int32_t relu, const float* h,
                             const float* s_src, const float* s_dst, const float* row_ms, const float* a_src,
                             const float* a_dst, const int32_t* rowptr_t, const int32_t* csr_src,
                             const int32_t* rowptr_s, const int32_t* csr_dst, float* dh, float* da_src, float* da_dst,
                             float* dbias, int32_t n, const int32_t* d_n, int32_t f, const int32_t* items_t,
                             const int32_t* d_n_items_t, const int32_t* items_s, const int32_t* d_n_items_s,
                             int32_t item_cap, void* workspace, int32_t* status, grapes_stream_t stream);

size_t grapes_gatv2_aggregate_workspace_bytes(int32_t item_cap, int32_t f, int32_t heads);
int grapes_gatv2_aggregate_fwd(const float* x_l, const float* x_r, const float* att, const int32_t* rowptr_t,
                               const int32_t* csr_src, const float* bias, float* out, float* agg, float* row_ms, int32_t n,
                               const int32_t* d_n, int32_t heads, int32_t c, int32_t concat, float negative_slope, int32_t relu,
                               const int32_t* long_items, const int32_t* d_n_items, int32_t item_cap, void* workspace,
                               int32_t* status, grapes_stream_t stream);
size_t grapes_gatv2_aggregate_bwd_workspace_bytes(int32_t n, int32_t item_cap, int32_t f, int32_t heads);
int grapes_gatv2_aggregate_bwd(const float* dout, const float* out, const float* agg, const float* bias, int32_t relu,
                               const float* x_l, const float* x_r, const float* att, const float* row_ms,
                               const int32_t* rowptr_t, const int32_t* csr_src, const int32_t* rowptr_s, const int32_t* csr_dst,
                               float* dx_l, float* dx_r, float* datt, float* dbias, int32_t n, const int32_t* d_n, int32_t heads,
                               int32_t c, int32_t concat, float negative_slope, const int32_t* items_t,
                               const int32_t* d_n_items_t, const int32_t* items_s, const int32_t* d_n_items_s, int32_t item_cap,
                               void* workspace, int32_t* status, grapes_stream_t stream);

int grapes_gcn2_loop_counts(const int32_t* edge_src, const int32_t* edge_dst, int32_t e, const int32_t* d_e,
                            const int32_t* node_map, int32_t n, const int32_t* d_n, int32_t* loops, grapes_stream_t stream);
int grapes_gcn2_loop_counts_csr(const int64_t* rowptr, const int32_t* col, int32_t n, int32_t* loops, grapes_stream_t stream);
size_t grapes_gcn2_propagate_workspace_bytes(int32_t n, int32_t item_cap, int32_t f);
int grapes_gcn2_propagate_fwd(const float* x, const float* x0, const int32_t* loops, const int32_t* rowptr_t,
                              const int32_t* csr_src, float alpha, float* s_out, float* p_out, int32_t n, const int32_t* d_n,
                              int32_t f, const int32_t* long_items, const int32_t* d_n_items, int32_t item_cap,
                              void* workspace, int32_t* status, grapes_stream_t stream);
int grapes_gcn2_propagate_bwd(const float* ds, const float* ds_add, int32_t add_is_p, const float* dx0_add, const int32_t* loops,
                              const int32_t* rowptr_s, const int32_t* csr_dst, float alpha, float* dx, float* dx0,
                              int32_t accumulate_x0, int32_t n, const int32_t* d_n, int32_t f, const int32_t* items_s,
                              const int32_t* d_n_items_s, int32_t item_cap, void* workspace, int32_t* status,
                              grapes_stream_t stream);
int grapes_gcn2_mix_fwd(const float* s, const float* t1, const float* t2, float c0, float c1, float c2, int32_t relu, float* out,
                        int32_t n, const int32_t* d_n, int32_t f, grapes_stream_t stream);
int grapes_gcn2_mix_bwd(const float* dout, const float* out, int32_t relu, float c0, float c1, float c2, float* g0, float* g1,
                        float* g2, int32_t n, const int32_t* d_n, int32_t f, grapes_stream_t stream);

size_t grapes_wgcn_structure_workspace_bytes(int32_t e);
int grapes_wgcn_structure(const int32_t* edge_src, const int32_t* edge_dst, int32_t e, const int32_t* d_e, int32_t n,
                          const int32_t* d_n, const int32_t* rowptr_t, const int32_t* csr_src, const int32_t* rowptr_s,
                          const int32_t* csr_dst, int32_t* pos_t, int32_t* pos_s, int32_t* inv_t, int32_t* inv_s,
                          int32_t* loop_src, void* workspace, int32_t* status, grapes_stream_t stream);
#define GRAPES_WGCN_LOOP_FILL 0
#define GRAPES_WGCN_LOOP_SUM 1
#define GRAPES_WGCN_UNNORMALIZED 2
size_t grapes_wgcn_loops_workspace_bytes(int32_t n, int32_t e);
int grapes_wgcn_loops(const int32_t* edge_src, const int32_t* edge_dst, int32_t e, const int32_t* d_e, int32_t n, const int32_t* d_n,
                      int32_t* loop_ptr, int32_t* loop_idx, void* workspace, grapes_stream_t stream);
int grapes_wgcn_weights(const float* edge_weight, int32_t e, const int32_t* inv_t, const int32_t* inv_s, const int32_t* loop_src,
                        const int32_t* loop_ptr, const int32_t* loop_idx, const int32_t* rowptr_t, const int32_t* rowptr_s, int32_t n,
                        const int32_t* d_n, int32_t mode, float fill, float* val_t, float* val_s, float* lw, float* dinv,
                        grapes_stream_t stream);
size_t grapes_wgcn_aggregate_workspace_bytes(int32_t item_cap, int32_t f);
int grapes_wgcn_aggregate_fwd(const float* h, const int32_t* rowptr_t, const int32_t* csr_src, const float* val_t, const float* dinv,
                              const float* lw, const float* bias, float* out, int32_t n, const int32_t* d_n, int32_t f,
                              int32_t relu, int32_t mode, const int32_t* long_items, const int32_t* d_n_items, int32_t item_cap,
                              void* workspace, int32_t* status, grapes_stream_t stream);
size_t grapes_wgcn_aggregate_bwd_workspace_bytes(int32_t n, int32_t e, int32_t item_cap, int32_t f);
int grapes_wgcn_aggregate_bwd(const float* dout, const float* relu_out, const float* h, const int32_t* edge_src,
                              const int32_t* edge_dst, int32_t e, const int32_t* d_e, const int32_t* pos_t, const int32_t* loop_src,
                              const int32_t* rowptr_t, const int32_t* csr_src, const float* val_t, const int32_t* rowptr_s,
                              const int32_t* csr_dst, const float* val_s, const float* dinv, const float* lw, float* dh,
                              float* dbias, float* dw, int32_t n, const int32_t* d_n, int32_t f, int32_t mode,
                              const int32_t* items_t, const int32_t* d_n_items_t, const int32_t* items_s,
                              const int32_t* d_n_items_s, int32_t item_cap, void* workspace, int32_t* status, grapes_stream_t stream);

size_t grapes_pna_aggregate_fwd_workspace_bytes(int32_t item_cap, int32_t f);
int grapes_pna_aggregate_fwd(const float* x, const float* a, const float* b, int32_t ld, const int32_t* loops,
                             const int32_t* rowptr_t, const int32_t* csr_src, int32_t n_agg, int32_t agg_code, int32_t n_scal,
// ... 333 lines not shown
```

Baseline: 512.9 million.

## Fuse GCN aggregate backward with input-gradient GEMM and batch weight-gradient slabs

Adds a kernel that performs the GCN backward aggregation (gated gather over sampled edges) and, in the same block, multiplies the aggregated rows by W with MFMA to produce the input gradient directly. The intermediate aggregated tile is kept in LDS rather than being re-read from global memory by a separate GEMM. The classifier backward loop now folds layers through this path and collects the weight-gradient slab jobs, issuing them as a single multi-problem launch. This cuts kernel launches and intermediate traffic on small sampled graphs. The cost is a more complex control flow with fallbacks and extra LDS use per block.

Measured after the change: 523.1 million (median of 6 runs). 2.0% higher.

```diff
diff --git a/grapes_amd/_lib.py b/grapes_amd/_lib.py
--- a/grapes_amd/_lib.py
+++ b/grapes_amd/_lib.py
@@ -223,6 +223,7 @@
     "grapes_linear_bwd_weight_slabs_bytes": (SZ, [I32, I32, I32]),
     "grapes_linear_bwd_weight_slabs": (I32, [P, P, P, I32, P, I32, I32, I32, P, P]),
     "grapes_linear_bwd_weight_slabs_and_input": (I32, [P, P, P, P, P, I32, P, I32, I32, I32, P, P]),
+    "grapes_linear_bwd_weight_slabs_multi": (I32, [I32, P, P, P, I32, P, P, P, P, P, P]),
     "grapes_slab_reduce_sets": (I32, [I32, P, P, P, I32, P, I32, P]),
     "grapes_gcn_aggregate_narrow_pair": (I32, [P, P, P, P, P, P, P, P, P, I32, P, P]),
     "grapes_linear_relu_head_fwd_bits": (I32, [P, I32, P, P, P, P, P, I32, P, I32, I32, P]),
@@ -246,6 +247,8 @@
     "grapes_gcn_aggregate_bwd_rank1_bits_multi": (I32, [I32, P, P, P, P, P, P, P, P, P, P, P, P, P, I32, P, P, P, P, P]),
     "grapes_gcn_aggregate_bwd_workspace_bytes": (SZ, [I32, I32]),
     "grapes_gcn_aggregate_bwd": (I32, [P, P, P, P, P, P, P, P, I32, I32, P, I32, P, P, I32, P, P, P]),
+    "grapes_gcn_aggregate_bwd_input_available": (I32, [P, P, P, I32, I32, I32]),
+    "grapes_gcn_aggregate_bwd_input": (I32, [P, P, P, P, P, P, P, P, P, I32, I32, P, I32, I32, P, P, P]),
     "grapes_sampler_workspace_bytes": (SZ, [I32]),
     "grapes_gumbel_topk": (I32, [P, P, P, U64, U64, P, I32, P, I32, I32, P, P, P, P, P, P, P, P, P, I32, P, P, P, P]),
     "grapes_gumbel_topk_hist": (I32, [P, P, P, U64, U64, P, I32, P, I32, I32, P, P, P, P, P, P, P, P, P, I32, P, P, P, P, P]),
diff --git a/grapes_amd/csrc/common.h b/grapes_amd/csrc/common.h
--- a/grapes_amd/csrc/common.h
+++ b/grapes_amd/csrc/common.h
@@ -363,7 +363,8 @@
 #include <string.h>
 enum GrapesRiderKind { GRAPES_RK_OTHER = 0, GRAPES_RK_EXPAND, GRAPES_RK_COMPACT, GRAPES_RK_FILL, GRAPES_RK_SORT, GRAPES_RK_GATHER,
                        GRAPES_RK_BEGIN ,
-                       GRAPES_RK_AGGBWD  };
+                       GRAPES_RK_AGGBWD ,
+                       GRAPES_RK_AGGBWD_DX  };
 struct GrapesRiderRecord {
     int kind = GRAPES_RK_OTHER, variant = 0, grid = 0, block = 0;
     size_t arg_bytes = 0;
diff --git a/grapes_amd/csrc/gemm_kernels.hip b/grapes_amd/csrc/gemm_kernels.hip
--- a/grapes_amd/csrc/gemm_kernels.hip
+++ b/grapes_amd/csrc/gemm_kernels.hip
@@ -1403,6 +1403,20 @@
         gemm_skinny_body<true>(b.A, b.B, b.C, n_host, d_n, b.N, b.K, b.lda, b.ldb, b.ldc, nullptr, 0, j % nb_x, j / nb_x, sk_smem);
     }
 }
+#define DWS_MULTI_MAX 4
+struct DwSmallSet { int count; DwSmallArgs p[DWS_MULTI_MAX]; int na_x[DWS_MULTI_MAX]; int start[DWS_MULTI_MAX + 1]; };
+__global__ __launch_bounds__(SK_T) void gemm_dw_small_multi_k(DwSmallSet st, int n_host, const int32_t* d_n) {
+    __shared__ __attribute__((aligned(16))) float dws_smem[DWS_SMEM_FLOATS];
+    const int id = blockIdx.x;
+    int q = 0;
+#pragma unroll
+    for (int u = 1; u < DWS_MULTI_MAX; ++u) if (u < st.count && id >= st.start[u]) q = u;
+#define DSEL(f) (q == 0 ? st.f[0] : (q == 1 ? st.f[1] : (q == 2 ? st.f[2] : st.f[3])))
+    const DwSmallArgs a = DSEL(p);
+    const int na_x = DSEL(na_x), j = id - DSEL(start);
+#undef DSEL
+    gemm_dw_small_body(a.A, a.gate, a.X, a.slabs, a.cs_slabs, n_host, d_n, a.M, a.N, a.lda, a.ldb, j % na_x, j / na_x, dws_smem);
+}
 static inline int dw_nslab(int f_out, int f_in);
 static inline bool dw_small_ok(int n, int f_out, int f_in) {
     return n <= 4096 && grapes_div_up(n, DWS_ROWS) <= dw_nslab(f_out, f_in);
@@ -1498,6 +1512,32 @@
     SkinnyArgs b{dout, w, dx, f_in, f_out, (long long)f_out, (long long)f_in, (long long)f_in};
     hipLaunchKernelGGL(gemm_dw_small_dx_pair_k, dim3(na_x * na_y + nb_x * nb_y), dim3(SK_T), lds_use, (hipStream_t)stream, a, b, n, d_n,
                        na_x, na_y, nb_x);
+    GRAPES_LAUNCH_CHECK();
+    return 0;
+}
+extern "C" int grapes_linear_bwd_weight_slabs_multi(int32_t count, const float* const* dout, const float* const* gate,
+                                                    const float* const* x, int32_t n, const int32_t* d_n, const int32_t* f_in,
+                                                    const int32_t* f_out, const int32_t* want_bias, void* const* workspace,
+                                                    grapes_stream_t stream) {
+    if (count < 1 || count > DWS_MULTI_MAX || !dout || !gate || !x || !f_in || !f_out || !want_bias || !workspace || n <= 0)
+        return GRAPES_EINVAL;
+    DwSmallSet st{}; st.count = count;
+    const size_t ns = (size_t)grapes_div_up(n, DWS_ROWS);
+    int total = 0;
+    for (int q = 0; q < DWS_MULTI_MAX; ++q) {
+        const int r = q < count ? q : 0;
+        if (q < count) {
+            if (f_in[r] <= 0 || f_out[r] <= 1 || !dout[r] || !x[r] || !workspace[r] || !dw_small_ok(n, f_out[r], f_in[r])) return GRAPES_EINVAL;
+        }
+        float* w_dw = (float*)workspace[r];
+        float* w_db = w_dw + ns * (size_t)f_in[r] * f_out[r];
+        st.p[q] = DwSmallArgs{dout[r], gate[r], x[r], w_dw, want_bias[r] ? w_db : nullptr, f_out[r], f_in[r], (long long)f_out[r], (long long)f_in[r]};
+        st.na_x[q] = grapes_div_up(f_out[r], SK_ROWS) * grapes_div_up(f_in[r], SK_COLS);
+        st.start[q] = total;
+        if (q < count) total += st.na_x[q] * (int)ns;
+    }
+    st.start[DWS_MULTI_MAX] = total;
+    hipLaunchKernelGGL(gemm_dw_small_multi_k, dim3(total), dim3(SK_T), 0, (hipStream_t)stream, st, n, d_n);
     GRAPES_LAUNCH_CHECK();
     return 0;
 }
diff --git a/grapes_amd/csrc/spmm_kernels.hip b/grapes_amd/csrc/spmm_kernels.hip
--- a/grapes_amd/csrc/spmm_kernels.hip
+++ b/grapes_amd/csrc/spmm_kernels.hip
@@ -1651,6 +1651,190 @@
     gcn_aggregate_bwd_small_body<VEC>(a, (int)blockIdx.x, (int)gridDim.x);
 }
 
+#define AD_ROWS 32
+#define AD_COLS 64
+#define AD_LDA (2 * AD_ROWS + 2)
+#define AD_PS_FLOATS (4 * 2 * 16 * 64)
+typedef float ad_f32x16 __attribute__((ext_vector_type(16)));
+struct AggBwdDxArgs { AggBwdSmallArgs a; const float* W; float* dx; int N; };
+static inline size_t agg_bwd_dx_lds_bytes(int F) {
+    const size_t img = (size_t)((F + 3) / 4) * 2 * AD_LDA;
+    return (img > AD_PS_FLOATS ? img : (size_t)AD_PS_FLOATS) * sizeof(float);
+}
+static inline int agg_bwd_dx_grid(const AggBwdDxArgs& p) {
+    return (p.a.dbias ? p.a.ncb * p.a.R : 0) + grapes_div_up(p.a.n_host, AD_ROWS) * grapes_div_up(p.N, AD_COLS);
+}
+template <int VEC>
+__device__ __forceinline__ void gcn_aggregate_bwd_dx_body(const AggBwdDxArgs& p, int BID, float* __restrict__ smem) {
+    const AggBwdSmallArgs& a = p.a;
+    const int F = a.F, N = p.N;
+    const int ncs = a.dbias ? a.ncb * a.R : 0;
+    if (BID < ncs) {
+        colsum_ticket_body(a.dout, a.gate, nullptr, nullptr, a.partials, a.dbias, a.n_host, a.d_n, F, a.accumulate_bias, a.ticket,
+                           BID % a.ncb, BID / a.ncb, a.R);
+        return;
+    }
+    constexpr int PER = VEC == 4 ? 16 : 4;
+    constexpr int IB = VEC == 4 ? 4 : 8;
+    const int nct = (N + AD_COLS - 1) / AD_COLS;
+    const int id = BID - ncs;
+    const int rt = id / nct, ctile = id - rt * nct;
+    const int m0 = rt * AD_ROWS, n0 = ctile * AD_COLS;
+    if (m0 >= a.n_host) return;
+    const int tid = threadIdx.x, lane = tid & 63, wid = __builtin_amdgcn_readfirstlane(tid >> 6);
+    const int li = lane & 31, h = lane >> 5;
+    const int KQ = (F + 3) >> 2;
+    const int per = (KQ + 3) >> 2;
+    const int kq0 = wid * per, kq1 = (kq0 + per < KQ) ? kq0 + per : KQ;
+    const float* __restrict__ W = p.W;
+    float bx[PER][2], by[PER][2];
+#pragma unroll
+    for (int i = 0; i < PER; ++i) {
+        const int kq = kq0 + i < KQ ? kq0 + i : KQ - 1;
+        const int k0 = 4 * kq + h, k1 = k0 + 2;
+#pragma unroll
+        for (int c = 0; c < 2; ++c) {
+            const int gn = n0 + 32 * c + li;
+            const int gc = gn < N ? gn : 0;
+            bx[i][c] = W[(long long)(k0 < F ? k0 : 0) * N + gc];
+            by[i][c] = W[(long long)(k1 < F ? k1 : 0) * N + gc];
+        }
+    }
+    const int n = eff_count(a.d_n, a.n_host);
+    if (m0 >= n) return;
+    const float* __restrict__ dout = a.dout;
+    const int32_t* __restrict__ rowptr = a.rowptr; const int32_t* __restrict__ csr = a.csr; const float* __restrict__ dinv = a.dinv;
+    const bool has_g = a.gate != nullptr;
+    const float* __restrict__ gp = has_g ? a.gate : a.dout;
+    float* As = smem;
+    const int f0 = lane * VEC;
+    const bool fl = f0 < F;
+    const int fc = fl ? f0 : 0;
+    int beg[8], P[9]; float dc[8];
+    P[0] = 0;
+#pragma unroll
+    for (int i = 0; i < 8; ++i) {
+        const int r = m0 + wid + 4 * i;
+        const bool ok = r < n;
+        const int rc = ok ? r : 0;
+        const int b = rowptr[rc], e = rowptr[rc + 1];
+        dc[i] = dinv[rc];
+        beg[i] = b;
+        P[i + 1] = P[i] + (ok ? e - b + 1 : 0);
+    }
+    const int L = P[8];
+    auto emit = [&](int m, const float (&v)[VEC]) {
+#pragma unroll
+        for (int q = 0; q < VEC; ++q) {
+            const int k = f0 + q;
+            if (k < KQ * 4) As[((k >> 2) * 2 + (k & 1)) * AD_LDA + m * 2 + ((k >> 1) & 1)] = v[q];
+        }
+        if (ctile == 0 && fl) {
+            float* o = a.dh + (long long)(m0 + m) * F + f0;
+#pragma unroll
+            for (int q = 0; q < VEC; ++q) o[q] = v[q];
+        }
+    };
+    float acc[VEC];
+#pragma unroll
+    for (int q = 0; q < VEC; ++q) acc[q] = 0.f;
+    for (int c0 = 0; c0 < L; c0 += 64) {
+        const int t = c0 + lane;
+        int ri = 0, base = 0, rb = beg[0]; float rdc = dc[0];
+#pragma unroll
+        for (int i = 1; i < 8; ++i)
+            if (t >= P[i]) { ri = i; base = P[i]; rb = beg[i]; rdc = dc[i]; }
+        int rend = P[1];
+#pragma unroll
+        for (int i = 1; i < 8; ++i) if (ri == i) rend = P[i + 1];
+        const bool live = t < L;
+        const bool self = live && t == rend - 1;
+        const bool nb = live && !self;
+        int s = nb ? csr[rb + (t - base)] : (live ? m0 + wid + 4 * ri : 0);
+        float w = rdc * rdc;
+        if (nb) w = dinv[s] * rdc;
+        const int meta = ri | (self ? 8 : 0);
+        const int cnt = L - c0 < 64 ? L - c0 : 64;
+        for (int b0 = 0; b0 < cnt; b0 += IB) {
+            float val[IB][VEC], g[IB][VEC];
+#pragma unroll
+            for (int u = 0; u < IB; ++u) {
+                const int l = b0 + u < cnt ? b0 + u : b0;
+                const int su = __builtin_amdgcn_readlane(s, l);
+                ld_vec<VEC>(dout + (long long)su * F + fc, val[u]);
+                ld_vec<VEC>(gp + (long long)su * F + fc, g[u]);
+            }
+#pragma unroll
+            for (int u = 0; u < IB; ++u) {
+                if (b0 + u < cnt) {
+                    const float wu = __int_as_float(__builtin_amdgcn_readlane(__float_as_int(w), b0 + u));
+                    const int mu = __builtin_amdgcn_readlane(meta, b0 + u);
+#pragma unroll
+                    for (int q = 0; q < VEC; ++q) {
+                        const float x = (fl && (!has_g || g[u][q] > 0.f)) ? val[u][q] : 0.f;
+                        acc[q] = fmaf(wu, x, acc[q]);
+                    }
+                    if (mu & 8) {
+                        emit(wid + 4 * (mu & 7), acc);
+#pragma unroll
+                        for (int q = 0; q < VEC; ++q) acc[q] = 0.f;
+                    }
+                }
+            }
+        }
+    }
+#pragma unroll
+    for (int i = 0; i < 8; ++i)
+        if (m0 + wid + 4 * i >= n) {
+#pragma unroll
+            for (int q = 0; q < VEC; ++q) {
+                const int k = f0 + q;
+                if (k < KQ * 4) As[((k >> 2) * 2 + (k & 1)) * AD_LDA + (wid + 4 * i) * 2 + ((k >> 1) & 1)] = 0.f;
+            }
+        }
+    __syncthreads();
+    ad_f32x16 acc0 = {0}, acc1 = {0};
+    {
+        const float* Ap = As + h * AD_LDA + li * 2;
+        const bool c0ok = n0 + li < N, c1ok = n0 + 32 + li < N;
+#pragma unroll
+        for (int i = 0; i < PER; ++i) {
+            const int kq = kq0 + i;
+            if (kq < kq1) {
+                const float2 av = *reinterpret_cast<const float2*>(Ap + (size_t)kq * 2 * AD_LDA);
+                const bool k0ok = 4 * kq + h < F, k1ok = 4 * kq + h + 2 < F;
+                acc0 = __builtin_amdgcn_mfma_f32_32x32x2f32(av.x, (k0ok && c0ok) ? bx[i][0] : 0.f, acc0, 0, 0, 0);
+                acc0 = __builtin_amdgcn_mfma_f32_32x32x2f32(av.y, (k1ok && c0ok) ? by[i][0] : 0.f, acc0, 0, 0, 0);
+                acc1 = __builtin_amdgcn_mfma_f32_32x32x2f32(av.x, (k0ok && c1ok) ? bx[i][1] : 0.f, acc1, 0, 0, 0);
+                acc1 = __builtin_amdgcn_mfma_f32_32x32x2f32(av.y, (k1ok && c1ok) ? by[i][1] : 0.f, acc1, 0, 0, 0);
+            }
+        }
+    }
+    __syncthreads();
+    float* Ps = smem;
+#pragma unroll
+    for (int r = 0; r < 16; ++r) {
+        Ps[((wid * 2 + 0) * 16 + r) * 64 + lane] = acc0[r];
+        Ps[((wid * 2 + 1) * 16 + r) * 64 + lane] = acc1[r];
+    }
+    __syncthreads();
+#pragma unroll
+    for (int u = 0; u < 8; ++u) {
+        const int o = tid + 256 * u;
+        const int ln = o & 63, r = (o >> 6) & 15, ct = o >> 10;
+        const float v0 = Ps[((0 * 2 + ct) * 16 + r) * 64 + ln], v1 = Ps[((1 * 2 + ct) * 16 + r) * 64 + ln];
+        const float v2 = Ps[((2 * 2 + ct) * 16 + r) * 64 + ln], v3 = Ps[((3 * 2 + ct) * 16 + r) * 64 + ln];
+        const int gn = n0 + 32 * ct + (ln & 31);
+        const int gm = m0 + (r & 3) + 8 * (r >> 2) + 4 * (ln >> 5);
+        if (gm < n && gn < N) p.dx[(long long)gm * N + gn] = ((v0 + v1) + v2) + v3;
+    }
+}
+template <int VEC>
+__global__ __launch_bounds__(256) void gcn_aggregate_bwd_dx_k(AggBwdDxArgs p) {
+    extern __shared__ __attribute__((aligned(16))) float ad_smem[];
+    gcn_aggregate_bwd_dx_body<VEC>(p, (int)blockIdx.x, ad_smem);
+}
+
 size_t grapes_colsum_workspace_bytes(int F) { return (size_t)CS_BLOCKS * (F > 0 ? F : 1) * sizeof(float); }
 
 int grapes_colsum_launch(const float* src, const float* gate, const float* wrow, float* dst, float* out, int n,
@@ -2113,6 +2297,36 @@
     float* partials = workspace ? (float*)((char*)workspace + grapes_colsum_workspace_bytes(f)) : nullptr;
     return launch_aggregate(dpre_buf, rowptr_s, csr_dst, dinv, nullptr, dh, n, d_n, f, 0, long_items, d_n_items, item_cap,
                             partials, s);
+}
+
+extern "C" int grapes_gcn_aggregate_bwd_input_available(const float* dout, const float* relu_out, const float* dt, int32_t n,
+                                                        int32_t f, int32_t f_in) {
+    const bool vec = (f % 4 == 0) && grapes_aligned16(dout) && grapes_aligned16(dt) && (!relu_out || grapes_aligned16(relu_out));
+    return (n > 0 && n <= 2048 && f > 16 && f <= 64 * (vec ? 4 : 1) && f_in >= 1) ? 1 : 0;
+}
+extern "C" int grapes_gcn_aggregate_bwd_input(const float* dout, const float* relu_out, const int32_t* rowptr_s,
+                                              const int32_t* csr_dst, const float* dinv, const float* w, float* dt, float* dx,
+                                              float* dbias, int32_t accumulate_bias, int32_t n, const int32_t* d_n, int32_t f,
+                                              int32_t f_in, void* workspace, uint32_t* d_ticket, grapes_stream_t stream) {
+    if (!dout || !rowptr_s || !csr_dst || !dinv || !w || !dt || !dx) return GRAPES_EINVAL;
+    if (!grapes_gcn_aggregate_bwd_input_available(dout, relu_out, dt, n, f, f_in)) return GRAPES_EINVAL;
+    if (dbias && (!workspace || !d_ticket)) return GRAPES_EINVAL;
+    const bool vec = (f % 4 == 0) && grapes_aligned16(dout) && grapes_aligned16(dt) && (!relu_out || grapes_aligned16(relu_out));
+    const int VECW = vec ? 4 : 1;
+    const int ncb = grapes_div_up(f, 64);
+    int R = grapes_div_up(n, 64); if (R > CS_SMALL_R) R = CS_SMALL_R; if (R < 1) R = 1;
+    const AggBwdDxArgs A{{dout, relu_out, rowptr_s, csr_dst, dinv, dt, n, d_n, f, dbias, accumulate_bias, (float*)workspace,
+                          (unsigned*)d_ticket, ncb, R}, w, dx, f_in};
+    const int grid = agg_bwd_dx_grid(A);
+    const size_t lds = agg_bwd_dx_lds_bytes(f);
+    auto single = [=](hipStream_t st) {
+        if (vec) hipLaunchKernelGGL((gcn_aggregate_bwd_dx_k<4>), dim3(grid), dim3(256), lds, st, A);
+        else hipLaunchKernelGGL((gcn_aggregate_bwd_dx_k<1>), dim3(grid), dim3(256), lds, st, A);
+    };
+    if (grapes_rider_recording()) { grapes_rider_record(grapes_rider_make(GRAPES_RK_AGGBWD_DX, VECW, grid, 256, A, single)); return 0; }
+    single((hipStream_t)stream);
+    GRAPES_LAUNCH_CHECK();
+    return 0;
 }
 
 
@@ -2196,6 +2410,25 @@
     }
 }
 
+template <int VEC>
+__global__ __launch_bounds__(256) void bernoulli_aggdx_pair_k(BernSegs sg, BernArgs ba, int gx, AggBwdDxArgs b) {
+    extern __shared__ __attribute__((aligned(16))) float ad_smem[];
+    if ((int)blockIdx.x < gx) bernoulli_dense_multi_body(sg, ba, (int)blockIdx.x, gx);
+    else gcn_aggregate_bwd_dx_body<VEC>(b, ((int)blockIdx.x - gx) + (int)blockIdx.y * ((int)gridDim.x - gx), ad_smem);
+}
+template <int VEC>
+__global__ __launch_bounds__(256) void narrow_multi_aggdx_pair_k(NarrowSegs sg, int F, int narrow_lane_rows, int gx, AggBwdDxArgs b) {
+    extern __shared__ __attribute__((aligned(16))) float ad_smem[];
+    if ((int)blockIdx.x < gx) {
+        const int q = blockIdx.y;
+#define NSEL(f) (q == 0 ? sg.f[0] : (q == 1 ? sg.f[1] : (q == 2 ? sg.f[2] : sg.f[3])))
+        narrow_body(NSEL(h), NSEL(rowptr), NSEL(csr), NSEL(dinv), NSEL(bias), NSEL(out), NSEL(n_cap), NSEL(d_n), F, 0,
+                    narrow_lane_rows, (int)blockIdx.x, gx);
+#undef NSEL
+    } else
+        gcn_aggregate_bwd_dx_body<VEC>(b, ((int)blockIdx.x - gx) + (int)blockIdx.y * ((int)gridDim.x - gx), ad_smem);
+}
+
 extern "C" size_t grapes_sampler_head_bwd_multi_workspace_bytes(void) { return (size_t)4 * 32 * sizeof(float); }
 
 extern "C" int grapes_sampler_head_bwd_multi_phase(int32_t count, const float* const* logits, const float* const* mask,
@@ -2232,10 +2465,23 @@
         rx = grapes_div_up(r->grid, count);
         return true;
     };
-    AggBwdSmallArgs B; int vecw = 0, rx = 0;
+    auto rider_dx = [&](AggBwdDxArgs& D, int& vecw, int& rx) -> bool {
+        const GrapesRiderRecord* r = grapes_rider_match(GRAPES_RK_AGGBWD_DX, 4, 256, s);
+        vecw = 4;
+        if (!r) { r = grapes_rider_match(GRAPES_RK_AGGBWD_DX, 1, 256, s); vecw = 1; }
+        if (!r) return false;
+        memcpy(&D, r->args, sizeof D);
+        rx = grapes_div_up(r->grid, count);
+        return true;
+    };
+    AggBwdSmallArgs B; AggBwdDxArgs D; int vecw = 0, rx = 0;
     if (phase != 2) {
         const BernArgs ba{d_grad_scale, sum_out, accumulate_sum, (float*)workspace, (unsigned*)d_ticket, mean_sum_out};
-        if (rider(B, vecw, rx)) {
+        if (rider_dx(D, vecw, rx)) {
+            const size_t lds = agg_bwd_dx_lds_bytes(D.a.F);
+            if (vecw == 4) hipLaunchKernelGGL((bernoulli_aggdx_pair_k<4>), dim3(g1 + rx, count), dim3(256), lds, s, bs, ba, g1, D);
+            else hipLaunchKernelGGL((bernoulli_aggdx_pair_k<1>), dim3(g1 + rx, count), dim3(256), lds, s, bs, ba, g1, D);
+        } else if (rider(B, vecw, rx)) {
             if (vecw == 4) hipLaunchKernelGGL((bernoulli_aggbwd_pair_k<4>), dim3(g1 + rx, count), dim3(256), 0, s, bs, ba, g1, B);
             else hipLaunchKernelGGL((bernoulli_aggbwd_pair_k<1>), dim3(g1 + rx, count), dim3(256), 0, s, bs, ba, g1, B);
         } else
@@ -2244,7 +2490,11 @@
     }
     if (phase != 1) {
         int g2 = grapes_div_up(nmax, 256); if (g2 > 4096) g2 = 4096;
-        if (rider(B, vecw, rx)) {
+        if (rider_dx(D, vecw, rx)) {
+            const size_t lds = agg_bwd_dx_lds_bytes(D.a.F);
+            if (vecw == 4) hipLaunchKernelGGL((narrow_multi_aggdx_pair_k<4>), dim3(g2 + rx, count), dim3(256), lds, s, ns, 1, narrow_lane_rows_cfg(), g2, D);
+            else hipLaunchKernelGGL((narrow_multi_aggdx_pair_k<1>), dim3(g2 + rx, count), dim3(256), lds, s, ns, 1, narrow_lane_rows_cfg(), g2, D);
+        } else if (rider(B, vecw, rx)) {
             if (vecw == 4) hipLaunchKernelGGL((narrow_multi_aggbwd_pair_k<4>), dim3(g2 + rx, count), dim3(256), 0, s, ns, 1, narrow_lane_rows_cfg(), g2, B);
             else hipLaunchKernelGGL((narrow_multi_aggbwd_pair_k<1>), dim3(g2 + rx, count), dim3(256), 0, s, ns, 1, narrow_lane_rows_cfg(), g2, B);
         } else
diff --git a/grapes_amd/ops.py b/grapes_amd/ops.py
--- a/grapes_amd/ops.py
+++ b/grapes_amd/ops.py
@@ -799,6 +799,35 @@
             self.sets.append((ws, ws.data_ptr() + ns * fo * fi * 4, dbias, fo))
         return True
 
+    def try_add_multi(self, problems):
+        import ctypes as C
+        k = len(problems)
+        n, d_n = problems[0][2].shape[0], problems[0][5]
+        nsets = sum(2 if p[4] is not None else 1 for p in problems)
+        if not (1 <= k <= 4) or any(p[2].shape[0] != n or p[5] is not d_n for p in problems):
+            return False
+        if len(self.sets) + nsets > 8:
+            self.flush()
+        if self.sets and (self.n != n or (self.d_n is None) != (d_n is None) or
+                          (d_n is not None and self.d_n.data_ptr() != d_n.data_ptr()) or self.acc):
+            self.flush()
+        fis, fos = [p[2].shape[1] for p in problems], [p[0].shape[1] for p in problems]
+        wss = [_ws(lib().grapes_linear_bwd_weight_slabs_bytes(n, fi, fo), problems[0][2].device) for fi, fo in zip(fis, fos)]
+        arr = lambda ts: (C.c_void_p * k)(*[None if t is None else t.data_ptr() for t in ts])
+        ints = lambda vs: (C.c_int32 * k)(*vs)
+        rc = lib().grapes_linear_bwd_weight_slabs_multi(k, arr([p[0] for p in problems]), arr([p[1] for p in problems]),
+                                                        arr([p[2] for p in problems]), n, _p(d_n), ints(fis), ints(fos),
+                                                        ints([1 if p[4] is not None else 0 for p in problems]), arr(wss), _stream())
+        if rc != 0:
+            return False
+        ns = (n + 127) // 128
+        self.n, self.d_n, self.acc = n, d_n, False
+        for (dout, gate, x, dw, dbias, _), ws, fi, fo in zip(problems, wss, fis, fos):
+            self.sets.append((ws, ws.data_ptr(), dw, fo * fi))
+            if dbias is not None:
+                self.sets.append((ws, ws.data_ptr() + ns * fo * fi * 4, dbias, fo))
+        return True
+
     def flush(self):
         if not self.sets:
             return
@@ -1258,6 +1287,7 @@
 
 
 _BWD_HOSTS: List = []
+_BWD_ALONE = [0]
 
 
 def carry_backward_aggregations(hosts):
@@ -1306,6 +1336,49 @@
         if alone < 0:
             raise _lib.GrapesHipError(f"rider_detach failed ({alone})")
     return dh, dbias
+
+
+def gcn_aggregate_bwd_input(dout, prep: PreparedGraph, w, relu_out=None, dbias=None, accumulate_bias=False, dt=None, dx=None):
+    _chk(dout, _f32, "dout"); _chk(relu_out, _f32, "relu_out", True); _chk(w, _f32, "w"); _chk(dbias, _f32, "dbias", True)
+    n, f = dout.shape
+    fi = w.shape[1]
+    dev = dout.device
+    if w.shape[0] != f or prep.n > _SMALL_GRAPH:
+        return None
+    _chk(dt, _f32, "dt", True); _chk(dx, _f32, "dx", True)
+    if dt is None:
+        dt = torch.empty_like(dout)
+    L = lib()
+    if not L.grapes_gcn_aggregate_bwd_input_available(_p(dout), _p(relu_out), _p(dt), n, f, fi):
+        return None
+    if dx is None:
+        dx = torch.empty((n, fi), dtype=_f32, device=dev)
+    if tuple(dt.shape) != (n, f) or tuple(dx.shape) != (n, fi):
+        raise ValueError("gcn_aggregate_bwd_input: dt [n, f], dx [n, f_in]")
+    ws = _ws(L.grapes_gcn_aggregate_bwd_workspace_bytes(0, f), dev)
+    host = _BWD_HOSTS.pop(0) if _BWD_HOSTS else None
+    if host is not None:
+        _lib.check(L.grapes_rider_record_begin(), "rider_record_begin")
+    prog = -1
+    try:
+        rc = L.grapes_gcn_aggregate_bwd_input(_p(dout), _p(relu_out), _p(prep.rowptr_s), _p(prep.csr_dst), _p(prep.dinv), _p(w),
+                                              _p(dt), _p(dx), _p(dbias), 1 if accumulate_bias else 0, n, _p(prep.d_n), f, fi,
+                                              _p(ws), _p(_ticket(dev)[16:32]), _stream())
+    finally:
+        if host is not None:
+            prog = int(L.grapes_rider_record_end())
+    _lib.check(rc, "gcn_aggregate_bwd_input")
+    if host is not None:
+        _lib.check(L.grapes_rider_attach(prog, 0, _stream()), "rider_attach")
+        try:
+            host()
+        finally:
+            alone = L.grapes_rider_detach(_stream(), None)
+            L.grapes_rider_free(prog)
+        if alone < 0:
+            raise _lib.GrapesHipError(f"rider_detach failed ({alone})")
+        _BWD_ALONE[0] += alone
+    return dt, dx
 
 
 def gather_width_ok(f: int, wide_scalar: bool = False) -> bool:
diff --git a/grapes_amd/step_graph.py b/grapes_amd/step_graph.py
--- a/grapes_amd/step_graph.py
+++ b/grapes_amd/step_graph.py
@@ -796,9 +796,37 @@
         layers, acts, used, keeps, alln, d_na = s.layers, s.acts, s.used, s.keeps, s.alln, s.d_na
         d = s.dl
         deferred = ops.DeferredSlabs() if _sw("GRAPES_DEFER_SLABS", "1") != "0" else None
+        fold = (deferred is not None and not self.embed and all(k is None for k in keeps) and
+                _sw("GRAPES_CLS_BWD_FOLD", "1") != "0")
+        slab_jobs = []
+
+        def flush_jobs():
+            if slab_jobs and not deferred.try_add_multi(slab_jobs):
+                for dout, gate, x, dw, dbias, dn in slab_jobs:
+                    if gate is None and dbias is None:
+                        ops.linear_bwd_weight(dout, x, d_n=dn, out=dw, accumulate=False, defer=deferred)
+                    else:
+                        ops.linear_bwd_weight_gated(dout, x, gate=gate, d_n=dn, dw=dw, dbias=dbias, accumulate=False,
+                                                    want_bias=dbias is not None, defer=deferred)
+            del slab_jobs[:]
+
         for i in range(len(layers) - 1, -1, -1):
             if keeps[i] is not None:
                 d = ops.dropout_bwd(d, keeps[i], self.dropout, d_n=d_na)
+            if fold and i == 0 and s.first_fused and self._fl[id(layers[0])].agg_first and slab_jobs:
+                fl0 = self._fl[id(layers[0])]
+                slab_jobs.append((d, acts[1] if s.first_relu else None, acts[0], fl0.grad, layers[0].bias.grad, used[0].d_n))
+                continue
+            if fold and i > 0:
+                conv = layers[i]
+                if not slab_jobs or slab_jobs[-1][5] is used[i].d_n:
+                    r = ops.gcn_aggregate_bwd_input(d, used[i], conv.lin.weight, relu_out=acts[i + 1] if i < len(layers) - 1 else None,
+                                                    dbias=conv.bias.grad, accumulate_bias=False)
+                    if r is not None:
+                        slab_jobs.append((r[0], None, acts[i], conv.lin.weight.grad, None, used[i].d_n))
+                        d = r[1]
+                        continue
+            flush_jobs()
             if i == 0 and s.first_fused:
                 self._first_bwd(layers[0], acts[0], acts[1], d, used[0], False, relu=s.first_relu, defer=deferred)
                 if self.embed:
@@ -811,6 +839,7 @@
             else:
                 d = self._conv_bwd(layers[i], acts[i], acts[i + 1], d, used[i], i < len(layers) - 1, i > 0, False,
                                    defer=deferred)
+        flush_jobs()
         if deferred is not None:
             if (self.grad_sync is None and self._fused_adam is not False and self.opt_c is not None and
                     not any(fl.publishes for fl in self._fl.values()) and not self.reinforce and
diff --git a/include/grapes_hip.h b/include/grapes_hip.h
--- a/include/grapes_hip.h
+++ b/include/grapes_hip.h
@@ -208,6 +208,9 @@
 int grapes_linear_bwd_weight_slabs_and_input(const float* dout, const float* gate, const float* x, const float* w, float* dx,
                                              int32_t n, const int32_t* d_n, int32_t f_in, int32_t f_out, int32_t want_bias,
                                              void* workspace, grapes_stream_t stream);
+int grapes_linear_bwd_weight_slabs_multi(int32_t count, const float* const* dout, const float* const* gate, const float* const* x,
+                                         int32_t n, const int32_t* d_n, const int32_t* f_in, const int32_t* f_out,
+                                         const int32_t* want_bias, void* const* workspace, grapes_stream_t stream);
 int grapes_slab_reduce_sets(int32_t nsets, const float* const* slabs, float* const* outs, const int64_t* counts, int32_t n,
                             const int32_t* d_n, int32_t accumulate, grapes_stream_t stream);
 int grapes_linear_relu_head_fwd_bits(const float* x, int32_t x_stride, const float* w, const float* bias,
@@ -314,6 +317,12 @@
                              const int32_t* d_n, int32_t f, const int32_t* long_items,
                              const int32_t* d_n_items, int32_t item_cap, void* workspace,
                              uint32_t* d_ticket, grapes_stream_t stream);
+int grapes_gcn_aggregate_bwd_input_available(const float* dout, const float* relu_out, const float* dt, int32_t n, int32_t f,
+                                             int32_t f_in);
+int grapes_gcn_aggregate_bwd_input(const float* dout, const float* relu_out, const int32_t* rowptr_s, const int32_t* csr_dst,
+                                   const float* dinv, const float* w, float* dt, float* dx, float* dbias,
+                                   int32_t accumulate_bias, int32_t n, const int32_t* d_n, int32_t f, int32_t f_in,
+                                   void* workspace, uint32_t* d_ticket, grapes_stream_t stream);
 
 int grapes_gat_scores(const float* h, const float* a_src, const float* a_dst, float* s_src, float* s_dst, int32_t n,
                       const int32_t* d_n, int32_t f, grapes_stream_t stream);
```
